# letao1991/EAD-GAN

Measured on NVIDIA B200. Metric: train images/sec (G+D+E step, 64x64 CelebA), higher is better.
Workload: dtype bf16

## Files before the change

eadgan_b200/_lib.py:

```python
from __future__ import annotations

import ctypes as C
import os

import torch

_HERE = os.path.dirname(os.path.abspath(__file__))
LIB_PATH = os.path.join(_HERE, "lib", "libeadgan.so")

ACT_NONE, ACT_RELU, ACT_LRELU, ACT_TANH, ACT_SIGMOID = 0, 1, 2, 3, 4
F32, BF16 = 0, 1
ADAM_MAX_TENSORS = 48


class Tensor4(C.Structure):
    _fields_ = [("ptr", C.c_void_p), ("sn", C.c_int64), ("sc", C.c_int64), ("sh", C.c_int64),
                ("sw", C.c_int64), ("dtype", C.c_int32), ("_pad", C.c_int32)]


class ConvDesc(C.Structure):
    _fields_ = [("n", C.c_int32), ("c", C.c_int32), ("h", C.c_int32), ("w", C.c_int32),
                ("k", C.c_int32), ("r", C.c_int32), ("s", C.c_int32), ("p", C.c_int32),
                ("q", C.c_int32), ("stride", C.c_int32), ("pad", C.c_int32)]


class TcDesc(C.Structure):
    _fields_ = [("n", C.c_int32), ("c", C.c_int32), ("h", C.c_int32), ("w", C.c_int32),
                ("k", C.c_int32), ("act", C.c_int32), ("slope", C.c_float),
                ("out_f32_nchw", C.c_int32), ("want_stats", C.c_int32), ("c_real", C.c_int32),
                ("mask_mode", C.c_int32)]


class AdamTensors(C.Structure):
    _fields_ = [("p", C.c_void_p * ADAM_MAX_TENSORS), ("g", C.c_void_p * ADAM_MAX_TENSORS),
                ("m", C.c_void_p * ADAM_MAX_TENSORS), ("v", C.c_void_p * ADAM_MAX_TENSORS),
                ("numel", C.c_int64 * ADAM_MAX_TENSORS), ("count", C.c_int32), ("_pad", C.c_int32)]


_P = C.c_void_p
_T4 = C.POINTER(Tensor4)
_I, _F, _D, _L = C.c_int, C.c_float, C.c_double, C.c_int64

_PROTOS = {
    "eadgan_conv_fprop": [C.POINTER(ConvDesc), _T4, _P, _P, _I, _F, _T4, _T4, _I, _F, _P],
    "eadgan_conv_dgrad": [C.POINTER(ConvDesc), _T4, _P, _P, _I, _F, _T4, _T4, _I, _F, _P],
    "eadgan_conv_wgrad": [C.POINTER(ConvDesc), _T4, _T4, _P, _P, C.c_size_t, _P],
    "eadgan_channel_sum": [_T4, _I, _I, _I, _I, _P, _P],
    "eadgan_tc_pack_w_fprop": [_P, _P, _I, _I, _I, _P, _P],
    "eadgan_tc_pack_w_dgrad": [_P, _P, _I, _I, _I, _P, _P],
    "eadgan_tc_dense_pack": [_P, _I, _I, _I, _I, _P, _P],
    "eadgan_tc_dense_gather": [_P, _P, _P, _P, _I, _I, _I, _P, C.c_size_t, _P],
    "eadgan_tc_dense_scatter": [_P, _P, _P, _P, _P, _I, _F, _I, _I, _I, _P, _P],
    "eadgan_tc_dense_wgrad": [_P, _P, _P, _P, C.c_size_t, _I, _I, _I, _I, _P],
    "eadgan_tc_fprop": [C.POINTER(TcDesc), _P, _P, _P, _P, _P, _P, _P, _P],
    "eadgan_tc_dgrad": [C.POINTER(TcDesc), _P, _P, _P, _P, _P, _P, _P, _P],
    "eadgan_tc_wgrad": [C.POINTER(TcDesc), _P, _P, _P, _P, C.c_size_t, _P],
    "eadgan_tc_gemm": [_P, _P, _P, _I, _I, _I, _P],
    "eadgan_tc_thin_expand": [_T4, _T4, _I, _F, _I, _I, _I, _I, _P, _P],
    "eadgan_tc_thin_pack_w": [_P, _I, _I, _I, _P, _P],
    "eadgan_tc_thin_fprop": [C.POINTER(TcDesc), _P, _P, _P, _P, _P, _P, _P, _P],
    "eadgan_tc_thin_wgrad": [C.POINTER(TcDesc), _P, _P, _P, _P, C.c_size_t, _P],
    "eadgan_tc_thin_dgrad": [C.POINTER(TcDesc), _P, _P, _P, _P, _P, _P],
    "eadgan_copy4": [_T4, _T4, _I, _I, _I, _I, _P],
    "eadgan_bn_stats": [_T4, _I, _I, _I, _I, _P, _P],
    "eadgan_bn_finalize": [_P, _D, _I, _F, _F, _P, _P, _P, _P, _P],
    "eadgan_bn_apply": [_T4, _I, _I, _I, _I, _P, _P, _P, _P, _I, _F, _T4, _P],
    "eadgan_bn_bwd_reduce": [_T4, _T4, _T4, _I, _I, _I, _I, _P, _P, _P, _P, _I, _F, _P, _P],
    "eadgan_bn_bwd_apply": [_T4, _T4, _T4, _I, _I, _I, _I, _P, _P, _P, _P, _I, _F, _P, _D, _T4, _P],
    "eadgan_bn_bwd_finalize": [_P, _P, _P, _D, _D, _P, _P, _P, _I, _P, _P, _P, _P],
    "eadgan_bn_eval": [_T4, _I, _I, _I, _I, _P, _P, _F, _P, _P, _I, _F, _T4, _P],
    "eadgan_act_fwd": [_P, _P, _L, _I, _F, _P],
    "eadgan_act_bwd": [_P, _P, _P, _L, _I, _F, _P],
    "eadgan_softmax_fwd": [_P, _P, _I, _I, _P],
    "eadgan_softmax_bwd": [_P, _P, _P, _I, _I, _P],
    "eadgan_upsample2x_fwd": [_P, _P, _I, _I, _I, _P],
    "eadgan_upsample2x_bwd": [_P, _P, _I, _I, _I, _P],
    "eadgan_spectral_norm_fwd": [_P, _I, _I, _P, _P, _I, _F, _P, _P, _P, _P],
    "eadgan_spectral_norm_scale": [_P, _P, _P, C.c_longlong, _P],
    "eadgan_spectral_norm_bwd": [_P, _P, _P, _P, _P, _I, _I, _P, _P, _P],
    "eadgan_bce_fwd": [_P, _P, _L, _P, _P],
    "eadgan_bce_bwd": [_P, _P, _P, _L, _P, _P],
    "eadgan_mse_fwd": [_P, _P, _L, _P, _P],
    "eadgan_mse_bwd": [_P, _P, _P, _L, _P, _P, _P],
    "eadgan_ce_fwd": [_P, _P, _I, _I, _P, _P],
    "eadgan_ce_bwd": [_P, _P, _P, _I, _I, _P, _P],
    "eadgan_mi_fwd": [_P, _P, _I, _I, _P, _P],
    "eadgan_mi_bwd": [_P, _P, _P, _I, _I, _P, _P],
    "eadgan_adam_step": [C.POINTER(AdamTensors), _D, _D, _D, _D, _D, _F, _P],
    "eadgan_adam_step_dev": [C.POINTER(AdamTensors), _D, _D, _D, _D, _P, _F, _P],
    "eadgan_adam_advance": [_P, _P],
    "eadgan_fill_f32": [_P, _L, _F, _P],
    "eadgan_f64_to_f32": [_P, _P, _L, _P],
    "eadgan_zero_halo": [_P, _I, _I, _I, _I, _P],
    "eadgan_stn_fwd": [_P, _P, _I, _I, _I, _I, _I, _P, _P],
    "eadgan_affine_grid_fwd": [_P, _I, _I, _I, _P, _P],
    "eadgan_affine_grid_bwd": [_P, _I, _I, _I, _P, _P],
    "eadgan_grid_sample_fwd": [_P, _P, _I, _I, _I, _I, _I, _I, _I, _P, _P],
    "eadgan_grid_sample_bwd": [_P, _P, _P, _I, _I, _I, _I, _I, _I, _I, _P, _P, _P],
    "eadgan_relcode_dims": [_I, _P, _P],
    "eadgan_relcode_fwd": [_I, _P, C.c_longlong, _P, C.c_longlong, _I, _P, _P, _P],
    "eadgan_relcode_bwd": [_I, _P, _P, _I, _P, _P, _P],
    "eadgan_philox": [_I, C.c_ulonglong, _P, C.c_longlong, _I, C.c_longlong, C.c_longlong, C.c_longlong, _F, _F, _I, _P, _P],
}
_SPECIAL = {
    "eadgan_last_error": ([], C.c_char_p),
    "eadgan_version": ([], C.c_int),
    "eadgan_sm_count": ([], C.c_int),
    "eadgan_kernel_launches": ([], C.c_int64),
    "eadgan_tc_workspace_bytes": ([C.POINTER(TcDesc), _I], C.c_size_t),
    "eadgan_conv_wgrad_workspace": ([C.POINTER(ConvDesc)], C.c_size_t),
    "eadgan_tc_thin_buffer_elems": ([_I, _I, _I], C.c_size_t),
    "eadgan_tc_dense_gather_workspace": ([_I], C.c_size_t),
    "eadgan_tc_thin_wgrad_workspace": ([C.POINTER(TcDesc)], C.c_size_t),
    "eadgan_tc_dense_wgrad_workspace": ([_I, _I], C.c_size_t),
    "eadgan_spectral_norm_scratch_floats": ([_I, _I, _I], C.c_size_t),
}
EXPORTED = sorted(list(_PROTOS) + list(_SPECIAL))

weights_epoch = 0


def bump_weights_epoch():
    global weights_epoch
    weights_epoch += 1


step_serial = 0


def next_step_serial():
    global step_serial
    step_serial += 1
    return step_serial


_lib = None
launches = 0


def lib():
    global _lib
    if _lib is None:
        if not os.path.exists(LIB_PATH):
            raise RuntimeError(
                f"{LIB_PATH} is missing: build it with `python -m eadgan_b200.build` "
                "(nvcc, sm_100a). eadgan_b200 has no CPU or cuDNN fallback.")
        l = C.CDLL(LIB_PATH)
        for name, args in _PROTOS.items():
            fn = getattr(l, name)
            fn.argtypes = args
            fn.restype = C.c_int
        for name, (args, res) in _SPECIAL.items():
            fn = getattr(l, name)
            fn.argtypes = args
            fn.restype = res
        _lib = l
    return _lib


_prof = None


def _flops(name, args):
    try:
        d = args[0]._obj
    except AttributeError:
        return 0
    if isinstance(d, ConvDesc):
        return 2 * d.n * d.p * d.q * d.k * d.c * d.r * d.s
    if isinstance(d, TcDesc):
        return 2 * d.n * (d.h // 2) * (d.w // 2) * d.k * d.c * 16
    return 0


def _shape_tag(args):
    try:
        d = args[0]._obj
    except (AttributeError, IndexError):
        return ""
    if isinstance(d, ConvDesc):
        return f"[n{d.n} c{d.c} h{d.h} k{d.k} r{d.r} s{d.stride}]"
    if isinstance(d, TcDesc):
        return f"[n{d.n} c{d.c} h{d.h} k{d.k}]"
    return ""


def profile_start():
    global _prof
    _prof = []


def profile_stop():
    global _prof
    rec, _prof = _prof, None
    torch.cuda.synchronize()
    out = {}
    for name, fl, e0, e1 in rec or []:
        r = out.setdefault(name, {"calls": 0, "ms": 0.0, "flops": 0})
        r["calls"] += 1
        r["ms"] += e0.elapsed_time(e1)
        r["flops"] += fl
    return out


def call(name, *args):
    global launches
    if _prof is not None:
        e0, e1 = torch.cuda.Event(enable_timing=True), torch.cuda.Event(enable_timing=True)
        e0.record()
        rc = getattr(lib(), name)(*args)
        e1.record()
        _prof.append((name + _shape_tag(args), _flops(name, args), e0, e1))
    else:
        rc = getattr(lib(), name)(*args)
    launches += 1
    if rc != 0:
        msg = lib().eadgan_last_error()
        raise RuntimeError(f"{name} failed ({rc}): {msg.decode() if msg else '?'}")


def stream():
    return C.c_void_p(torch.cuda.current_stream().cuda_stream)


def ptr(t):
    return None if t is None else C.c_void_p(t.data_ptr())


def _dt(t):
    if t.dtype == torch.float32:
        return F32
    if t.dtype == torch.bfloat16:
        return BF16
    raise RuntimeError(f"eadgan_b200: unsupported dtype {t.dtype}")


def t4(t: torch.Tensor) -> Tensor4:
    if t.dim() == 2:
        return Tensor4(t.data_ptr(), t.stride(0), t.stride(1), 0, 0, _dt(t), 0)
    assert t.dim() == 4, t.shape
    return Tensor4(t.data_ptr(), t.stride(0), t.stride(1), t.stride(2), t.stride(3), _dt(t), 0)


def require_cuda(t: torch.Tensor, who: str):
    if not t.is_cuda:
        raise RuntimeError(
            f"{who}: eadgan_b200 operators run only on CUDA tensors (sm_100a kernels, no CPU "
            f"fallback); got a {t.device} tensor")
```

eadgan_b200/chain.py:

```python
from __future__ import annotations

import ctypes as C
import os

import torch

from . import _lib as L
from . import functional as Fn
from . import tc
from ._lib import ACT_NONE, call, ptr, stream, t4


def precision():
    return os.environ.get("EADGAN_PRECISION", "bf16")


gate_log = None


def _pow2(v):
    return v > 0 and (v & (v - 1)) == 0


class _Stage:
    __slots__ = ("kind", "conv", "bn", "act", "stride", "pad", "r")

    def __init__(self, kind, conv):
        self.kind, self.conv, self.bn, self.act = kind, conv, None, (ACT_NONE, 0.0)
        self.stride = conv.stride[0]
        self.pad = conv.padding[0]
        self.r = conv.kernel_size[0]


def _compile(seq):
    from . import nn as enn
    mods = list(seq._modules.values())
    stages, i = [], 0
    while i < len(mods):
        m = mods[i]
        if isinstance(m, enn.Conv2d):
            kind = "conv"
        elif isinstance(m, enn.ConvTranspose2d):
            kind = "convT"
        else:
            return None
        if (m.groups != 1 or m.dilation != (1, 1) or m.kernel_size[0] != m.kernel_size[1]
                or m.stride[0] != m.stride[1] or m.padding[0] != m.padding[1] or m._forward_hooks
                or m._backward_hooks or getattr(m, "padding_mode", "zeros") != "zeros"
                or (kind == "convT" and m.output_padding != (0, 0))):
            return None
        st = _Stage(kind, m)
        i += 1
        if i < len(mods) and isinstance(mods[i], enn.BatchNorm2d) and enn._plain(mods[i]):
            bn = mods[i]
            if not (bn.affine and bn.track_running_stats) or bn.momentum is None:
                return None
            st.bn = bn
            i += 1
        if i < len(mods) and isinstance(mods[i], enn._Act) and enn._plain(mods[i]):
            st.act = mods[i].act()
            i += 1
        stages.append(st)
    if not stages or stages[-1].bn is not None:
        return None
    return stages


def _plan(seq):
    key = tuple(id(m) for m in seq._modules.values())
    cached = seq.__dict__.get("_eadgan_plan")
    if cached is None or cached[0] != key:
        cached = (key, _compile(seq))
        seq.__dict__["_eadgan_plan"] = cached
    return cached[1]


_sn_streams = {}
prefetch_enabled = True


def _side_stream(dev):
    side = _sn_streams.get(dev)
    if side is None:
        side = _sn_streams[dev] = torch.cuda.Stream(device=dev)
    side.wait_stream(torch.cuda.current_stream())
    return side


def prefetch_spectral_norm(seq, count=1):
    if precision() != "bf16" or not prefetch_enabled:
        return
    stages = _plan(seq)
    if stages is None:
        return
    convs = [st.conv for st in stages if st.conv._forward_pre_hooks]
    if not convs:
        return
    w0 = getattr(convs[0], "weight_orig", None)
    if w0 is None or not w0.is_cuda:
        return
    side = _side_stream(w0.device)
    with torch.cuda.stream(side):
        for _ in range(count):
            done = []
            Fn.sn_skip_scale = True
            try:
                for conv in convs:
                    conv.__dict__.pop("_eadgan_sn_src", None)
                    for hook in conv._forward_pre_hooks.values():
                        hook(conv, (None,))
                    done.append((conv.weight, conv.__dict__.get("_eadgan_sn_src")))
            finally:
                Fn.sn_skip_scale = False
            ev = torch.cuda.Event()
            ev.record(side)
            for conv, entry in zip(convs, done):
                tag = getattr(getattr(conv, "weight_orig", None), "_eadgan_stepped", 0)
                conv.__dict__.setdefault("_eadgan_sn_queue", []).append((entry, ev, tag))


def prefetch_packs(module):
    if precision() != "bf16" or not prefetch_enabled:
        return
    todo = []
    for seq in module.modules():
        if not isinstance(seq, torch.nn.Sequential):
            continue
        stages = _plan(seq)
        if stages is None:
            continue
        for st in stages:
            p = getattr(st.conv, "weight_orig", None)
            if p is None:
                p = st.conv.weight
            if isinstance(p, torch.nn.Parameter) and p.is_cuda and getattr(p, "_eadgan_pack_uses", None):
                todo.append(p)
    if not todo:
        return
    with torch.cuda.stream(_side_stream(todo[0].device)):
        for p in todo:
            tc.prefetch_packs(p)


def set_trainable(module, flag):
    for p in module.parameters():
        p.requires_grad_(flag)


def clear_prefetch(seq):
    for m in seq._modules.values():
        m.__dict__.pop("_eadgan_sn_queue", None)


def try_run(seq, x):
    if precision() != "bf16" or not torch.is_tensor(x) or not x.is_cuda or x.dim() != 4 or x.dtype != torch.float32:
        return None
    stages = _plan(seq)
    if stages is None:
        return None
    if any(st.bn is not None and not st.bn.training for st in stages):
        return None
    params, srcs = [], []
    for st in stages:
        queue = st.conv.__dict__.get("_eadgan_sn_queue")
        if queue:
            (w_pre, sn_pre), ev, tag = queue.pop(0)
            if tag != getattr(getattr(st.conv, "weight_orig", None), "_eadgan_stepped", 0):
                raise RuntimeError("eadgan_b200.chain: a prefetched spectral-norm result is older than the layer's "
                                   "weights (an optimiser stepped them after prefetch_spectral_norm); the step driver "
                                   "must prefetch only forwards that run before the owning optimiser steps")
            cur = torch.cuda.current_stream()
            cur.wait_event(ev)
            for t in (w_pre,) + (tuple(sn_pre[1:3]) if sn_pre is not None else ()):
                if torch.is_tensor(t):
                    t.record_stream(cur)
            setattr(st.conv, "weight", w_pre)
            if sn_pre is not None:
                st.conv.__dict__["_eadgan_sn_src"] = sn_pre
            else:
                st.conv.__dict__.pop("_eadgan_sn_src", None)
        else:
            st.conv.__dict__.pop("_eadgan_sn_src", None)
            Fn.sn_skip_scale = True
            try:
                for hook in st.conv._forward_pre_hooks.values():
                    hook(st.conv, (x,))
            finally:
                Fn.sn_skip_scale = False
        w = st.conv.weight
        sn = st.conv.__dict__.get("_eadgan_sn_src")
        if sn is not None and sn[2] is w and isinstance(sn[0], torch.nn.Parameter):
            srcs.append((sn[0], sn[1], sn[3]))
        elif sn is not None and sn[3]:
            Fn.spectral_norm_materialize(sn[0], sn[1], sn[2])
            srcs.append(None)
        elif isinstance(w, torch.nn.Parameter):
            srcs.append((w, None))
        else:
            srcs.append(None)
        params += [w, st.conv.bias]
        if st.bn is not None:
            st.bn.num_batches_tracked.add_(1)
            params += [st.bn.weight, st.bn.bias]
    if gate_log is not None:
        gate_log.append((seq, []))
    return _ChainFn.apply(x, stages, srcs, *params)


class _Buf:
    __slots__ = ("t", "fmt")

    def __init__(self, t, fmt):
        self.t, self.fmt = t, fmt

    @property
    def nchw(self):
        if self.fmt == "ext":
            return tuple(self.t.shape)
        n, hp, wp, c = self.t.shape
        return (n, c, hp - 2, wp - 2)

    def view(self):
        return self.t if self.fmt == "ext" else tc.interior(self.t)

    def padded(self):
        return self.t if self.fmt == "pad" else tc.to_padded(self.t)


def _geom(st, in_shape):
    w = st.conv.weight
    r, s_, pad = st.r, st.stride, st.pad
    if st.kind == "conv":
        n, c, h, ww = in_shape
        k = w.shape[0]
        p = (h + 2 * pad - r) // s_ + 1
        q = (ww + 2 * pad - r) // s_ + 1
    else:
        n, k, p, q = in_shape
        c = w.shape[1]
        h = (p - 1) * s_ - 2 * pad + r
        ww = (q - 1) * s_ - 2 * pad + r
    return L.ConvDesc(n, c, h, ww, k, r, r, p, q, s_, pad)


def _calloc(d):
    if d.c % 32 == 0:
        return d.c
    return 32 if d.c < 32 else None


def _tc_ok(d, direction):
    if not (d.r == 4 and d.stride == 2 and d.pad == 1 and d.h == 2 * d.p and d.w == 2 * d.q):
        return False
    if not (_pow2(d.p) and _pow2(d.q)) or _calloc(d) is None:
        return False
    if direction == "fprop":
        return d.k % 32 == 0 and d.q <= 128
    if direction == "dgrad":
        return (d.k % 64 == 0 or d.k == 32) and d.q <= 128
    return d.k % 32 == 0 and d.q <= 64


def _thin_ok(d, direction):
    if not (d.r == 4 and d.stride == 2 and d.pad == 1 and d.h == 2 * d.p and d.w == 2 * d.q and d.c <= 4):
        return False
    if not (_pow2(d.p) and _pow2(d.q)):
        return False
    if direction == "fprop":
        return d.k % 32 == 0 and d.q <= 128
    if direction == "dgrad":
        return (d.k % 64 == 0 or d.k == 32) and d.q == 32 and d.c <= 3
    return d.k % 32 == 0 and d.q <= 64


def _impl(st, d, last):
    unit = d.r == 4 and d.stride == 1 and d.pad == 0 and d.h == 4 and d.w == 4 and d.p == 1 and d.q == 1
    plain = st.bn is None and st.act[0] == ACT_NONE
    if unit and plain and d.c % 128 == 0:
        if st.kind == "convT" and d.k <= 256 and not last:
            return "dense_T"
        if st.kind == "conv" and d.k <= 32 and last:
            return "dense_C"
    direction = "fprop" if st.kind == "conv" else "dgrad"
    if _thin_ok(d, direction) and (st.kind == "conv" or (last and st.bn is None)):
        return "thin"
    if _tc_ok(d, direction):
        if _calloc(d) != d.c and st.kind == "convT" and not (last and st.bn is None):
            return "simt"
        return "tc"
    return "simt"


class _StagePlan:
    __slots__ = ("d", "ca", "fwd", "wgrad", "dx", "fuse", "in_fmt", "out_fmt", "in_shape", "out_shape")


def _plan_kernels(stages, in_shape):
    plans = []
    for si, st in enumerate(stages):
        last, conv = si == len(stages) - 1, st.kind == "conv"
        prev = stages[si - 1] if si > 0 else None
        p = _StagePlan()
        d = p.d = _geom(st, in_shape)
        p.in_shape = tuple(in_shape)
        p.out_shape = (d.n, d.k, d.p, d.q) if conv else (d.n, d.c, d.h, d.w)
        p.fwd = _impl(st, d, last)
        p.ca = _calloc(d) if p.fwd == "tc" else d.c
        if p.fwd in ("dense_T", "dense_C"):
            p.wgrad = "dense"
            p.dx = "dense" if p.fwd == "dense_C" and si > 0 else "simt"
        elif p.fwd == "thin":
            if conv and last:
                raise RuntimeError("eadgan_b200.chain: a thin conv cannot be the last stage")
            p.wgrad = "thin" if _thin_ok(d, "wgrad") else "simt"
            if conv:
                p.dx = "thin" if si == 0 and _thin_ok(d, "dgrad") else "simt"
            else:
                p.dx = "thin" if si > 0 else "simt"
        elif p.fwd == "tc":
            p.wgrad = "tc" if _tc_ok(d, "wgrad") else "simt"
            tc_dx = _tc_ok(d, "dgrad" if conv else "fprop") and not (conv and si > 0 and p.ca != d.c)
            p.dx = "tc" if tc_dx else "simt"
        else:
            p.wgrad = p.dx = "simt"
        p.in_fmt = "ext" if si == 0 and (p.fwd in ("dense_T", "simt") or (p.fwd == "thin" and conv)) else "pad"
        p.out_fmt = "ext" if last else "pad"
        p.fuse = prev is not None and prev.bn is None and prev.act[0] != ACT_NONE
        plans.append(p)
        in_shape = p.out_shape
    return plans


def _chan_sums(buf, c):
    n, cc, h, w = buf.nchw
    if buf.fmt == "ext" and h * w == 1 and cc == c and buf.t.dtype == torch.float32:
        return Fn.channel_sum(buf.t)
    sums = torch.zeros(2 * c, device=buf.t.device, dtype=torch.float64)
    d = t4(buf.view())
    call("eadgan_bn_stats", C.byref(d), n, c, h, w, ptr(sums), stream())
    return sums[:c].float()


def _r64(v):
    return (v + 63) // 64 * 64


class _Arena:

    def __init__(self, n, dev):
        self.buf = torch.zeros(n + 2, device=dev, dtype=torch.float64) if n > 0 else None
        self.off = 0

    def take(self, n):
        n2 = (n + 1) // 2 * 2
        if self.buf is None or self.off + n2 > self.buf.numel():
            return torch.zeros(n, device=self.buf.device if self.buf is not None else "cuda", dtype=torch.float64)
        out = self.buf[self.off:self.off + n]
        self.off += n2
        return out


class _Saved:
    __slots__ = ("w", "src", "lazy", "pi", "has_b", "inp", "y", "R", "a", "pre", "mean", "invstd", "gamma", "beta",
                 "count", "n_local", "sum_x")

    def __init__(self, w, src, pi, has_b):
        self.w, self.src, self.pi, self.has_b = w, src, pi, has_b
        self.lazy = src is not None and len(src) > 2 and bool(src[2])
        self.R = self.a = self.pre = None

    def values(self):
        if self.lazy:
            Fn.spectral_norm_materialize(self.src[0], self.src[1], self.w)
            self.lazy = False
        return self.w.contiguous()

    def packed(self, direction, ca):
        if self.src is not None:
            return tc.pack_w_cached(self.src[0], direction, ca), self.src[1]
        return tc.pack_w(self.values(), None, direction, ca), None

    def packed_thin(self, direction):
        if self.src is not None:
            return tc.thin_pack_w_cached(self.src[0], direction), self.src[1]
        return tc.thin_pack_w(self.values(), direction), None


class _ChainFn(torch.autograd.Function):
    @staticmethod
    def forward(ctx, x, stages, srcs, *params):
        st_ = stream()
        dev = x.device
        plans = _plan_kernels(stages, tuple(x.shape))
        cur = _Buf(x.contiguous(), "ext")
        saved = []
        pi = 0
        arena = _Arena(sum(2 * p.out_shape[1] for st, p in zip(stages, plans) if st.bn is not None), dev)
        for si, (st, p) in enumerate(zip(stages, plans)):
            sv = _Saved(params[pi], srcs[si], pi, params[pi + 1] is not None)
            b = params[pi + 1]
            pi += 4 if st.bn is not None else 2
            d, conv, last = p.d, st.kind == "conv", si == len(stages) - 1
            out_shape = p.out_shape
            cout = out_shape[1]
            epi_act = st.act if st.bn is None else (ACT_NONE, 0.0)
            stats = arena.take(2 * cout) if st.bn is not None else None
            inp = cur if cur.fmt == p.in_fmt else _Buf(tc.to_padded(cur.t, p.ca if conv else None), "pad")
            if p.fwd == "thin" and conv:
                sv.R = tc.thin_expand(inp.view())
                wpk, sg = sv.packed_thin("fprop")
                out_t = tc.thin_fprop(sv.R, wpk, b, d.c, cout, *epi_act, stats=stats, sigma=sg)
            elif p.fwd == "thin":
                wpk, sg = sv.packed_thin("dgrad")
                out_t = tc.thin_dgrad(inp.t, wpk, b, d.c, *epi_act, sigma=sg)
            elif p.fwd == "dense_T":
                sv.a = tc.pad_rows(inp.t.reshape(d.n, d.k), _r64(d.k))
                out_t = tc.dense_scatter(sv.a, tc.dense_pack(sv.values(), _r64(d.k), False), b, d.c)
            elif p.fwd == "dense_C":
                out_t = tc.dense_gather(inp.t, tc.dense_pack(sv.values(), 32, True), b, d.k).view(out_shape)
            elif p.fwd == "tc" and conv:
                wpk, sg = sv.packed("fprop", p.ca)
                out_t = tc.fprop(inp.t, wpk, b, cout, *epi_act, out_f32_nchw=last, stats=stats, sigma=sg)
            elif p.fwd == "tc":
                wpk, sg = sv.packed("dgrad", p.ca)
                out_t = tc.dgrad(inp.t, wpk, b, p.ca, *epi_act, out_f32_nchw=last, stats=stats,
                                 c_real=d.c if p.ca != d.c else 0, sigma=sg)
            else:
                out_t = (torch.empty(out_shape, device=dev, dtype=torch.float32) if last
                         else tc.alloc_padded(out_shape[0], out_shape[2], out_shape[3], cout, dev))
                ind, outd = t4(inp.view()), t4(out_t if last else tc.interior(out_t))
                call("eadgan_conv_fprop" if conv else "eadgan_conv_dgrad", C.byref(d), C.byref(ind),
                     ptr(sv.values()), ptr(b), epi_act[0], float(epi_act[1]), C.byref(outd), None, ACT_NONE, 0.0, st_)
                if stats is not None:
                    call("eadgan_bn_stats", C.byref(outd), out_shape[0], cout, out_shape[2], out_shape[3],
                         ptr(stats), st_)
            out = _Buf(out_t, p.out_fmt)
            sv.inp = inp
            if st.bn is not None:
                bn = st.bn
                gamma, beta = params[pi - 2], params[pi - 1]
                n_local = float(out_shape[0] * out_shape[2] * out_shape[3])
                count = n_local
                sum_x = stats
                if Fn._allreduce_sum is not None:
                    sum_x = stats[:cout].clone()
                    Fn._allreduce_sum(stats)
                    count *= Fn._world_size
                mean = torch.empty(cout, device=dev, dtype=torch.float32)
                invstd = torch.empty(cout, device=dev, dtype=torch.float32)
                call("eadgan_bn_finalize", ptr(stats), count, cout, float(bn.eps), float(bn.momentum), ptr(mean),
                     ptr(invstd), ptr(bn.running_mean), ptr(bn.running_var), st_)
                y = _Buf(tc.alloc_padded(out_shape[0], out_shape[2], out_shape[3], cout, dev), "pad")
                xd, yd = t4(out.view()), t4(y.view())
                call("eadgan_bn_apply", C.byref(xd), out_shape[0], cout, out_shape[2], out_shape[3], ptr(mean),
                     ptr(invstd), ptr(gamma), ptr(beta), st.act[0], float(st.act[1]), C.byref(yd), st_)
                sv.pre, sv.mean, sv.invstd, sv.gamma, sv.beta = out, mean, invstd, gamma, beta
                sv.count, sv.n_local, sv.sum_x = count, n_local, sum_x
                out = y
            sv.y = out
            if gate_log is not None and st.act[0] in (L.ACT_RELU, L.ACT_LRELU):
                gate_log[-1][1].append(out.view() > 0)
            saved.append(sv)
            cur = out
        saved[-1].y = None
        ctx.save_for_backward(cur.t)
        ctx.stages, ctx.plans, ctx.saved = stages, plans, saved
        return cur.t

    @staticmethod
    def backward(ctx, gout):
        stages, plans, saved = ctx.stages, ctx.plans, ctx.saved
        saved[-1].y = _Buf(ctx.saved_tensors[0], "ext")
        st_ = stream()
        dev = gout.device
        g = _Buf(gout.contiguous(), "ext")
        g_masked = False
        db_sums = None
        grads = []
        arena = _Arena(sum(3 * max(p.d.k, p.d.c) for p in plans), dev)
        for si in range(len(stages) - 1, -1, -1):
            st, p, sv = stages[si], plans[si], saved[si]
            d, conv = p.d, st.kind == "conv"
            n, cout, oh, ow = p.out_shape
            dgamma = dbeta = None
            need_dw = ctx.needs_input_grad[3 + sv.pi]
            need_db = sv.has_b and ctx.needs_input_grad[3 + sv.pi + 1]
            need_dx = si > 0 or ctx.needs_input_grad[0]
            if st.bn is not None:
                sums = arena.take(2 * cout)
                gd, xd, yd = t4(g.view()), t4(sv.pre.view()), t4(sv.y.view())
                call("eadgan_bn_bwd_reduce", C.byref(gd), C.byref(xd), C.byref(yd), n, cout, oh, ow, ptr(sv.mean),
                     ptr(sv.invstd), ptr(sv.gamma), ptr(sv.beta), st.act[0], float(st.act[1]), ptr(sums), st_)
                local = sums
                if Fn._allreduce_sum is not None:
                    local = sums.clone()
                    Fn._allreduce_sum(sums)
                call("eadgan_bn_bwd_apply", C.byref(gd), C.byref(xd), C.byref(yd), n, cout, oh, ow, ptr(sv.mean),
                     ptr(sv.invstd), ptr(sv.gamma), ptr(sv.beta), st.act[0], float(st.act[1]), ptr(sums),
                     float(sv.count), C.byref(gd), st_)
                small = torch.empty(3 * cout, device=dev, dtype=torch.float32)
                dgamma, dbeta, db_bn = small[:cout], small[cout:2 * cout], small[2 * cout:]
                call("eadgan_bn_bwd_finalize", ptr(local), ptr(sums), ptr(sv.sum_x), float(sv.n_local),
                     float(sv.count), ptr(sv.mean), ptr(sv.invstd), ptr(sv.gamma), cout, ptr(dgamma),
                     ptr(dbeta), ptr(db_bn) if sv.has_b else None, st_)
                dz = g
            elif st.act[0] != ACT_NONE and not g_masked:
                if g.fmt != "ext" or sv.y.fmt != "ext":
                    raise RuntimeError("eadgan_b200.chain: unfused activation backward on a private buffer")
                dz = _Buf(Fn.act_bwd(g.t, sv.y.t, st.act[0], st.act[1]), "ext")
            else:
                dz = g
            if not need_db:
                db = None
            elif st.bn is not None:
                db = db_bn
            elif db_sums is not None and dz is g:
                db = torch.empty(cout, device=dev, dtype=torch.float32)
                call("eadgan_f64_to_f32", ptr(db_sums), ptr(db), cout, st_)
            else:
                db = _chan_sums(dz, cout)
            db_sums = None
            want_sums = (si > 0 and stages[si - 1].bn is None and saved[si - 1].has_b
                         and ctx.needs_input_grad[3 + saved[si - 1].pi + 1] and p.in_shape[1] <= 1024)
            sums_buf = arena.take(p.in_shape[1]) if want_sums else None
            x_big, dy_small = (sv.inp, dz) if conv else (dz, sv.inp)
            r, a = sv.R, sv.a
            if p.fwd == "thin" and not conv and (need_dw or (need_dx and p.dx == "thin")):
                r = tc.thin_expand(dz.view())
            if p.fwd == "dense_C":
                a = tc.pad_rows(dz.t.reshape(d.n, d.k), 64)
            dw = None
            if not need_dw:
                pass
            elif p.wgrad == "thin":
                dw = tc.thin_wgrad(r, dy_small.padded(), d.c)
            elif p.wgrad == "dense":
                dw = tc.dense_wgrad(a, x_big.padded(), d.k)
            elif p.wgrad == "tc":
                xb = x_big.t if x_big.fmt == "pad" else tc.to_padded(x_big.t, p.ca)
                if not conv and p.ca != d.c:
                    dz = _Buf(xb, "pad")
                dw = tc.wgrad(xb, dy_small.padded(), c_real=d.c if p.ca != d.c else 0)
            else:
                dw = torch.empty_like(sv.w, memory_format=torch.contiguous_format)
                Fn.conv_wgrad(d, t4(x_big.view()), t4(dy_small.view()), dw)
            if need_dx:
                mask = sv.inp.t if p.fuse else None
                mask_act, mask_slope = stages[si - 1].act if p.fuse else (ACT_NONE, 0.0)
                if p.dx == "thin" and conv:
                    wpk, sg = sv.packed_thin("dgrad")
                    dx_t = tc.thin_dgrad(dz.padded(), wpk, None, d.c, sigma=sg)
                elif p.dx == "thin":
                    wpk, sg = sv.packed_thin("fprop")
                    dx_t = tc.thin_fprop(r, wpk, None, d.c, d.k, mask=mask, mask_mode=mask_act, slope=mask_slope,
                                         stats=sums_buf, stats_mode=2, sigma=sg)
                elif p.dx == "dense":
                    dx_t = tc.dense_scatter(a, tc.dense_pack(sv.values(), 64, False), None, d.c, mask=mask,
                                            mask_act=mask_act, slope=mask_slope, chan_sums=sums_buf)
                elif p.dx == "tc" and conv:
                    wpk, sg = sv.packed("dgrad", p.ca)
                    dx_t = tc.dgrad(dz.padded(), wpk, None, p.ca, mask=mask, mask_mode=mask_act, slope=mask_slope,
                                    out_f32_nchw=si == 0, c_real=d.c if p.ca != d.c else 0, stats=sums_buf,
                                    stats_mode=2, sigma=sg)
                elif p.dx == "tc":
                    wpk, sg = sv.packed("fprop", p.ca)
                    dzp = dz.t if dz.fmt == "pad" else tc.to_padded(dz.t, p.ca)
                    dx_t = tc.fprop(dzp, wpk, None, d.k, mask=mask, mask_mode=mask_act, slope=mask_slope,
                                    out_f32_nchw=si == 0, stats=sums_buf, stats_mode=2, sigma=sg)
                else:
                    ic, ih, iw = p.in_shape[1:]
                    dx_t = (tc.alloc_padded(d.n, ih, iw, ic, dev) if si > 0
                            else torch.empty(p.in_shape, device=dev, dtype=torch.float32))
                    dzd, dxd = t4(dz.view()), t4(dx_t if si == 0 else tc.interior(dx_t))
                    md = t4(sv.inp.view()) if p.fuse else None
                    call("eadgan_conv_dgrad" if conv else "eadgan_conv_fprop", C.byref(d), C.byref(dzd),
                         ptr(sv.values()), None, ACT_NONE, 0.0, C.byref(dxd), C.byref(md) if p.fuse else None,
                         mask_act, float(mask_slope), st_)
                g, g_masked = _Buf(dx_t, "ext" if si == 0 else "pad"), p.fuse
                db_sums = sums_buf if p.dx != "simt" else None
            stage_grads = [dw, db]
            if st.bn is not None:
                stage_grads += [dgamma, dbeta]
            grads = stage_grads + grads
        dx0 = g.t if ctx.needs_input_grad[0] else None
        ctx.saved = ctx.plans = None
        return (dx0, None, None, *grads)
```

eadgan_b200/csrc/spectral_norm.cu:

```cuda
#include "common.cuh"

namespace {

__global__ void __launch_bounds__(128) sn_wtu_kernel(const float* __restrict__ W, const float* __restrict__ u,
                                                     float* __restrict__ t, int rows, int cols, int rows_per_blk) {
  const int j = blockIdx.x * 128 + threadIdx.x;
  const int r0 = blockIdx.y * rows_per_blk;
  const int r1 = min(rows, r0 + rows_per_blk);
  if (j >= cols) return;
  float acc = 0.f;
  int i = r0;
  for (; i + 4 <= r1; i += 4) {
    const float a0 = W[(int64_t)i * cols + j], a1 = W[(int64_t)(i + 1) * cols + j];
    const float a2 = W[(int64_t)(i + 2) * cols + j], a3 = W[(int64_t)(i + 3) * cols + j];
    acc = fmaf(a0, u[i], acc); acc = fmaf(a1, u[i + 1], acc);
    acc = fmaf(a2, u[i + 2], acc); acc = fmaf(a3, u[i + 3], acc);
  }
  for (; i < r1; ++i) acc = fmaf(W[(int64_t)i * cols + j], u[i], acc);
  t[(int64_t)blockIdx.y * cols + j] = acc;
}

__global__ void __launch_bounds__(256) sn_vsum_kernel(float* __restrict__ t, int n, int parts, float* __restrict__ nrm) {
  __shared__ float red[32];
  const int i = blockIdx.x * 256 + threadIdx.x;
  float x = 0.f;
  if (i < n) {
    x = t[i];
    for (int p = 1; p < parts; ++p) x += t[(int64_t)p * n + i];
    t[i] = x;
  }
  const float s = eg_block_sum(x * x, red);
  if (threadIdx.x == 0) nrm[blockIdx.x] = s;
}

__global__ void __launch_bounds__(256) sn_wv_kernel(const float* __restrict__ W, const float* __restrict__ x,
                                                    const float* __restrict__ nrm, int nparts, float eps,
                                                    float* __restrict__ v, float* __restrict__ s, int rows, int cols) {
  __shared__ float red[32];
  const int i = blockIdx.x;
  const float* wr = W + (int64_t)i * cols;
  float inv = 1.f;
  if (x != nullptr) {
    float q = 0.f;
    for (int p = 0; p < nparts; ++p) q += nrm[p];
    inv = 1.f / fmaxf(sqrtf(q), eps);
    const int chunk = (cols + rows - 1) / rows;
    for (int j = i * chunk + threadIdx.x; j < min(cols, (i + 1) * chunk); j += blockDim.x) v[j] = x[j] * inv;
  }
  const float* src = x != nullptr ? x : v;
  float acc = 0.f;
  if ((cols & 3) == 0 && ((reinterpret_cast<uintptr_t>(wr) | reinterpret_cast<uintptr_t>(src)) & 15) == 0) {
    for (int j = threadIdx.x; j < (cols >> 2); j += blockDim.x) {
      const float4 a = reinterpret_cast<const float4*>(wr)[j];
      float4 b = reinterpret_cast<const float4*>(src)[j];
      if (x != nullptr) { b.x *= inv; b.y *= inv; b.z *= inv; b.w *= inv; }
      acc = fmaf(a.x, b.x, acc); acc = fmaf(a.y, b.y, acc);
      acc = fmaf(a.z, b.z, acc); acc = fmaf(a.w, b.w, acc);
    }
  } else {
    for (int j = threadIdx.x; j < cols; j += blockDim.x) acc = fmaf(wr[j], x != nullptr ? src[j] * inv : src[j], acc);
  }
  acc = eg_block_sum(acc, red);
  if (threadIdx.x == 0) s[i] = acc;
}

__global__ void __launch_bounds__(1024) sn_sigma_kernel(const float* __restrict__ s, float* __restrict__ u, int rows,
                                                        float eps, int update_u, float* __restrict__ sigma) {
  __shared__ float red[32];
  if (update_u) {
    float q = 0.f;
    for (int i = threadIdx.x; i < rows; i += blockDim.x) q = fmaf(s[i], s[i], q);
    q = eg_block_sum(q, red);
    const float inv = 1.f / fmaxf(sqrtf(q), eps);
    for (int i = threadIdx.x; i < rows; i += blockDim.x) u[i] = s[i] * inv;
    __syncthreads();
  }
  float d = 0.f;
  for (int i = threadIdx.x; i < rows; i += blockDim.x) d = fmaf(u[i], s[i], d);
  d = eg_block_sum(d, red);
  if (threadIdx.x == 0) *sigma = d;
}

__global__ void __launch_bounds__(256) sn_scale_kernel(const float* __restrict__ W, const float* __restrict__ sigma,
                                                       float* __restrict__ out, int64_t n) {
  const float sg = *sigma;
  const int64_t tid = blockIdx.x * (int64_t)blockDim.x + threadIdx.x, nth = (int64_t)gridDim.x * blockDim.x;
  if ((n & 3) == 0 && ((reinterpret_cast<uintptr_t>(W) | reinterpret_cast<uintptr_t>(out)) & 15) == 0) {
    for (int64_t i = tid; i < (n >> 2); i += nth) {
      float4 a = reinterpret_cast<const float4*>(W)[i];
      a.x /= sg; a.y /= sg; a.z /= sg; a.w /= sg;
      reinterpret_cast<float4*>(out)[i] = a;
    }
  } else {
    for (int64_t i = tid; i < n; i += nth) out[i] = W[i] / sg;
  }
}

__global__ void __launch_bounds__(256) sn_dot_kernel(const float* __restrict__ a, const float* __restrict__ b,
                                                     int64_t n, float* __restrict__ part) {
  __shared__ float red[32];
  float s = 0.f;
  if ((n & 3) == 0 && ((reinterpret_cast<uintptr_t>(a) | reinterpret_cast<uintptr_t>(b)) & 15) == 0) {
    for (int64_t i = blockIdx.x * (int64_t)blockDim.x + threadIdx.x; i < (n >> 2); i += (int64_t)gridDim.x * blockDim.x) {
      const float4 x = reinterpret_cast<const float4*>(a)[i], y = reinterpret_cast<const float4*>(b)[i];
      s = fmaf(x.x, y.x, s); s = fmaf(x.y, y.y, s); s = fmaf(x.z, y.z, s); s = fmaf(x.w, y.w, s);
    }
  } else {
    for (int64_t i = blockIdx.x * (int64_t)blockDim.x + threadIdx.x; i < n; i += (int64_t)gridDim.x * blockDim.x)
      s = fmaf(a[i], b[i], s);
  }
  s = eg_block_sum(s, red);
  if (threadIdx.x == 0) part[blockIdx.x] = s;
}

__global__ void __launch_bounds__(256) sn_bwd_kernel(const float* __restrict__ dW, const float* __restrict__ u,
                                                     const float* __restrict__ v, const float* __restrict__ sigma,
                                                     const float* __restrict__ part, int nparts, int rows, int cols,
                                                     float* __restrict__ out) {
  __shared__ float red[32];
  float d = 0.f;
  for (int i = threadIdx.x; i < nparts; i += blockDim.x) d += part[i];
  d = eg_block_sum(d, red);
  const float sg = *sigma;
  const float coef = d / (sg * sg);
  const int64_t n = (int64_t)rows * cols;
  if ((cols & 3) == 0 && ((reinterpret_cast<uintptr_t>(dW) | reinterpret_cast<uintptr_t>(out) | reinterpret_cast<uintptr_t>(v)) & 15) == 0) {
    const int cv = cols >> 2;
    for (int64_t i = blockIdx.x * (int64_t)blockDim.x + threadIdx.x; i < (n >> 2); i += (int64_t)gridDim.x * blockDim.x) {
      const int r = (int)(i / cv), c4 = (int)(i - (int64_t)r * cv);
      const float4 g = reinterpret_cast<const float4*>(dW)[i], vv = reinterpret_cast<const float4*>(v)[c4];
      const float cu = coef * u[r];
      float4 o;
      o.x = g.x / sg - cu * vv.x; o.y = g.y / sg - cu * vv.y; o.z = g.z / sg - cu * vv.z; o.w = g.w / sg - cu * vv.w;
      reinterpret_cast<float4*>(out)[i] = o;
    }
  } else {
    for (int64_t i = blockIdx.x * (int64_t)blockDim.x + threadIdx.x; i < n; i += (int64_t)gridDim.x * blockDim.x) {
      const int r = (int)(i / cols), c = (int)(i - (int64_t)r * cols);
      out[i] = dW[i] / sg - coef * u[r] * v[c];
    }
  }
}

constexpr int SN_SMALL_MAX = 16 * 1024;
constexpr int SN_SMALL_COLS = 4096, SN_SMALL_ROWS = 1024;
__global__ void __launch_bounds__(1024) sn_small_fwd_kernel(const float* __restrict__ W, float* __restrict__ u,
                                                            float* __restrict__ v, int rows, int cols, int do_pi, float eps,
                                                            float* __restrict__ sigma) {
  __shared__ float red[32];
  __shared__ float vs[SN_SMALL_COLS];
  __shared__ float ss[SN_SMALL_ROWS];
  const int tid = threadIdx.x, warp = tid >> 5, lane = tid & 31;
  if (do_pi) {
    for (int i = tid; i < rows; i += 1024) ss[i] = u[i];
    __syncthreads();
    float q = 0.f;
    for (int j = tid; j < cols; j += 1024) {
      float acc = 0.f;
#pragma unroll 8
      for (int i = 0; i < rows; ++i) acc = fmaf(W[(int64_t)i * cols + j], ss[i], acc);
      vs[j] = acc;
      q = fmaf(acc, acc, q);
    }
    q = eg_block_sum(q, red);
    const float inv = 1.f / fmaxf(sqrtf(q), eps);
    for (int j = tid; j < cols; j += 1024) { const float x = vs[j] * inv; vs[j] = x; v[j] = x; }
  } else {
    for (int j = tid; j < cols; j += 1024) vs[j] = v[j];
  }
  __syncthreads();
  for (int i = warp; i < rows; i += 32) {
    const float* wr = W + (int64_t)i * cols;
    float acc = 0.f;
#pragma unroll 8
    for (int j = lane; j < cols; j += 32) acc = fmaf(wr[j], vs[j], acc);
#pragma unroll
    for (int o = 16; o > 0; o >>= 1) acc += __shfl_xor_sync(0xffffffffu, acc, o);
    if (lane == 0) ss[i] = acc;
  }
  __syncthreads();
  if (do_pi) {
    float q = 0.f;
    for (int i = tid; i < rows; i += 1024) q = fmaf(ss[i], ss[i], q);
    q = eg_block_sum(q, red);
    const float inv = 1.f / fmaxf(sqrtf(q), eps);
    float d = 0.f;
    for (int i = tid; i < rows; i += 1024) { const float x = ss[i] * inv; u[i] = x; d = fmaf(x, ss[i], d); }
    d = eg_block_sum(d, red);
    if (tid == 0) *sigma = d;
  } else {
    float d = 0.f;
    for (int i = tid; i < rows; i += 1024) d = fmaf(u[i], ss[i], d);
    d = eg_block_sum(d, red);
    if (tid == 0) *sigma = d;
  }
}

__global__ void __launch_bounds__(1024) sn_small_bwd_kernel(const float* __restrict__ dW, const float* __restrict__ W,
                                                            const float* __restrict__ u, const float* __restrict__ v,
                                                            const float* __restrict__ sigma, int rows, int cols,
                                                            float* __restrict__ out) {
  __shared__ float red[32];
  const int n = rows * cols;
  float d = 0.f;
  for (int i = threadIdx.x; i < n; i += 1024) d = fmaf(dW[i], W[i], d);
  d = eg_block_sum(d, red);
  const float sg = *sigma;
  const float coef = d / (sg * sg);
  for (int i = threadIdx.x; i < n; i += 1024) {
    const int r = i / cols, c = i - r * cols;
    out[i] = dW[i] / sg - coef * u[r] * v[c];
  }
}

bool sn_small(int rows, int cols) {
  return (int64_t)rows * cols <= SN_SMALL_MAX && cols <= SN_SMALL_COLS && rows <= SN_SMALL_ROWS;
}

int grid_for(int64_t n) {
  int64_t b = (n + 1023) / 1024;
  const int64_t cap = 16 * (int64_t)eg_sm_count();
  return (int)(b < 1 ? 1 : (b > cap ? cap : b));
}

}

extern "C" int eadgan_spectral_norm_fwd(const float* w_orig, int rows, int cols, float* u, float* v,
                                        int do_power_iter, float eps, float* sigma, float* w_sn,
                                        float* scratch, void* stream) {
  EG_REQUIRE(w_orig && u && v && sigma && scratch && rows > 0 && cols > 0, EADGAN_ERR_INVALID,
             "spectral_norm_fwd: bad arguments");
  cudaStream_t st = (cudaStream_t)stream;
  if (sn_small(rows, cols)) {
    sn_small_fwd_kernel<<<1, 1024, 0, st>>>(w_orig, u, v, rows, cols, do_power_iter ? 1 : 0, eps, sigma);
    EG_LAUNCH_CHECK("sn_small_fwd_kernel");
    if (w_sn) {
      const int64_t n = (int64_t)rows * cols;
      sn_scale_kernel<<<grid_for(n), 256, 0, st>>>(w_orig, sigma, w_sn, n);
      EG_LAUNCH_CHECK("sn_scale_kernel");
    }
    return 0;
  }
  int col_tiles = (cols + 127) / 128;
  int splits = (4 * eg_sm_count() + col_tiles - 1) / col_tiles;
  int max_splits = (rows + 15) / 16;
  if (splits > max_splits) splits = max_splits;
  if (splits < 1) splits = 1;
  const int rpb = (rows + splits - 1) / splits;
  splits = (rows + rpb - 1) / rpb;
  float* s = scratch;
  float* nrm = scratch + ((rows + 3) & ~3);
  const int nparts = (cols + 255) / 256;
  float* t = nrm + ((nparts + 3) & ~3);
  if (do_power_iter) {
    sn_wtu_kernel<<<dim3(col_tiles, splits), 128, 0, st>>>(w_orig, u, t, rows, cols, rpb);
    EG_LAUNCH_CHECK("sn_wtu_kernel");
    sn_vsum_kernel<<<nparts, 256, 0, st>>>(t, cols, splits, nrm);
    EG_LAUNCH_CHECK("sn_vsum_kernel");
  }
  sn_wv_kernel<<<rows, 256, 0, st>>>(w_orig, do_power_iter ? t : nullptr, nrm, nparts, eps, v, s, rows, cols);
  EG_LAUNCH_CHECK("sn_wv_kernel");
  sn_sigma_kernel<<<1, 1024, 0, st>>>(s, u, rows, eps, do_power_iter ? 1 : 0, sigma);
  EG_LAUNCH_CHECK("sn_sigma_kernel");
  if (w_sn) {
    const int64_t n = (int64_t)rows * cols;
    sn_scale_kernel<<<grid_for(n), 256, 0, st>>>(w_orig, sigma, w_sn, n);
    EG_LAUNCH_CHECK("sn_scale_kernel");
  }
  return 0;
}

extern "C" int eadgan_spectral_norm_bwd(const float* dw_sn, const float* w_orig, const float* u,
                                        const float* v, const float* sigma, int rows, int cols,
                                        float* dw_orig, float* scratch, void* stream) {
  EG_REQUIRE(dw_sn && w_orig && u && v && sigma && dw_orig && scratch && rows > 0 && cols > 0,
             EADGAN_ERR_INVALID, "spectral_norm_bwd: bad arguments");
  cudaStream_t st = (cudaStream_t)stream;
  const int64_t n = (int64_t)rows * cols;
  if (sn_small(rows, cols)) {
    sn_small_bwd_kernel<<<1, 1024, 0, st>>>(dw_sn, w_orig, u, v, sigma, rows, cols, dw_orig);
    EG_LAUNCH_CHECK("sn_small_bwd_kernel");
    return 0;
  }
  const int parts = grid_for(n);
  sn_dot_kernel<<<parts, 256, 0, st>>>(dw_sn, w_orig, n, scratch);
  EG_LAUNCH_CHECK("sn_dot_kernel");
  sn_bwd_kernel<<<grid_for(n), 256, 0, st>>>(dw_sn, u, v, sigma, scratch, parts, rows, cols, dw_orig);
  EG_LAUNCH_CHECK("sn_bwd_kernel");
  return 0;
}

extern "C" size_t eadgan_spectral_norm_scratch_floats(int rows, int cols, int backward) {
  if (backward) return (size_t)grid_for((int64_t)rows * cols) + 8;
  return (size_t)((rows + 3) & ~3) + (size_t)(((cols + 255) / 256 + 3) & ~3) + (size_t)((rows + 15) / 16 + 1) * (size_t)cols + 8;
}

extern "C" int eadgan_spectral_norm_scale(const float* w_orig, const float* sigma, float* w_sn, long long n,
                                          void* stream) {
  EG_REQUIRE(w_orig && sigma && w_sn && n > 0, EADGAN_ERR_INVALID, "spectral_norm_scale: bad arguments");
  sn_scale_kernel<<<grid_for(n), 256, 0, (cudaStream_t)stream>>>(w_orig, sigma, w_sn, n);
  EG_LAUNCH_CHECK("sn_scale_kernel");
  return 0;
}
```

eadgan_b200/functional.py:

```python
from __future__ import annotations

import ctypes as C

import torch

from . import _lib as L
from . import tc
from ._lib import ACT_NONE, ACT_LRELU, ACT_RELU, ACT_SIGMOID, ACT_TANH, call, ptr, stream, t4

_allreduce_sum = None
_world_size = 1


def set_allreduce(fn, world_size):
    global _allreduce_sum, _world_size
    _allreduce_sum, _world_size = fn, int(world_size)


def _f32(t, who):
    L.require_cuda(t, who)
    if t.dtype != torch.float32:
        raise RuntimeError(f"{who}: expected float32, got {t.dtype}")
    return t


def _conv_desc(n, c, h, w, k, r, s, stride, pad):
    p = (h + 2 * pad - r) // stride + 1
    q = (w + 2 * pad - s) // stride + 1
    return L.ConvDesc(n, c, h, w, k, r, s, p, q, stride, pad), p, q


def act_fwd_(x, kind, slope=0.0, out=None):
    out = x if out is None else out
    call("eadgan_act_fwd", ptr(x), ptr(out), x.numel(), kind, float(slope), stream())
    return out


def act_bwd(dy, y, kind, slope=0.0):
    dy = dy.contiguous()
    dx = torch.empty_like(dy)
    call("eadgan_act_bwd", ptr(dy), ptr(y), ptr(dx), dy.numel(), kind, float(slope), stream())
    return dx


def channel_sum(t):
    if t.dim() == 2:
        n, c, h, w = t.shape[0], t.shape[1], 1, 1
    else:
        n, c, h, w = t.shape
    out = torch.empty(c, device=t.device, dtype=torch.float32)
    d = t4(t)
    call("eadgan_channel_sum", C.byref(d), n, c, h, w, ptr(out), stream())
    return out


def conv_wgrad(d, x_t4, dy_t4, dw):
    need = L.lib().eadgan_conv_wgrad_workspace(C.byref(d))
    ws = tc._workspace(need, dw.device) if need else None
    call("eadgan_conv_wgrad", C.byref(d), C.byref(x_t4), C.byref(dy_t4), ptr(dw), ptr(ws),
         C.c_size_t(need), stream())


class _ConvFn(torch.autograd.Function):

    @staticmethod
    def forward(ctx, x, w, b, stride, pad, act, slope):
        _f32(x, "conv2d")
        _f32(w, "conv2d")
        x = x if x.is_contiguous() else x.contiguous()
        w = w.contiguous()
        two_d = x.dim() == 2
        if two_d:
            n, c, h, ww = x.shape[0], x.shape[1], 1, 1
            k, r, s = w.shape[0], 1, 1
        else:
            n, c, h, ww = x.shape
            k, _, r, s = w.shape
        if w.shape[1] != c:
            raise RuntimeError(f"conv2d: weight {tuple(w.shape)} does not match input channels {c}")
        d, p, q = _conv_desc(n, c, h, ww, k, r, s, stride, pad)
        y = torch.empty((n, k) if two_d else (n, k, p, q), device=x.device, dtype=torch.float32)
        xd, yd = t4(x), t4(y)
        call("eadgan_conv_fprop", C.byref(d), C.byref(xd), ptr(w), ptr(b), act, float(slope),
             C.byref(yd), None, ACT_NONE, 0.0, stream())
        ctx.save_for_backward(x, w, y if act != ACT_NONE else None)
        ctx.cfg = (d, act, slope, b is not None)
        return y

    @staticmethod
    def backward(ctx, dy):
        x, w, y = ctx.saved_tensors
        d, act, slope, has_b = ctx.cfg
        dy = dy.contiguous()
        dz = act_bwd(dy, y, act, slope) if act != ACT_NONE else dy
        dx = dw = db = None
        dzd = t4(dz)
        if ctx.needs_input_grad[0]:
            dx = torch.empty_like(x)
            dxd = t4(dx)
            call("eadgan_conv_dgrad", C.byref(d), C.byref(dzd), ptr(w), None, ACT_NONE, 0.0,
                 C.byref(dxd), None, ACT_NONE, 0.0, stream())
        if ctx.needs_input_grad[1]:
            dw = torch.empty_like(w)
            conv_wgrad(d, t4(x), dzd, dw)
        if has_b and ctx.needs_input_grad[2]:
            db = channel_sum(dz)
        return dx, dw, db, None, None, None, None


class _ConvTFn(torch.autograd.Function):

    @staticmethod
    def forward(ctx, x, w, b, stride, pad, act, slope):
        _f32(x, "conv_transpose2d")
        _f32(w, "conv_transpose2d")
        x = x if x.is_contiguous() else x.contiguous()
        w = w.contiguous()
        n, k, p, q = x.shape
        kk, c, r, s = w.shape
        if kk != k:
            raise RuntimeError(f"conv_transpose2d: weight {tuple(w.shape)} does not match input channels {k}")
        h = (p - 1) * stride - 2 * pad + r
        ww = (q - 1) * stride - 2 * pad + s
        d = L.ConvDesc(n, c, h, ww, k, r, s, p, q, stride, pad)
        y = torch.empty((n, c, h, ww), device=x.device, dtype=torch.float32)
        xd, yd = t4(x), t4(y)
        call("eadgan_conv_dgrad", C.byref(d), C.byref(xd), ptr(w), ptr(b), act, float(slope),
             C.byref(yd), None, ACT_NONE, 0.0, stream())
        ctx.save_for_backward(x, w, y if act != ACT_NONE else None)
        ctx.cfg = (d, act, slope, b is not None)
        return y

    @staticmethod
    def backward(ctx, dy):
        x, w, y = ctx.saved_tensors
        d, act, slope, has_b = ctx.cfg
        dy = dy.contiguous()
        dz = act_bwd(dy, y, act, slope) if act != ACT_NONE else dy
        dx = dw = db = None
        dzd = t4(dz)
        if ctx.needs_input_grad[0]:
            dx = torch.empty_like(x)
            dxd = t4(dx)
            call("eadgan_conv_fprop", C.byref(d), C.byref(dzd), ptr(w), None, ACT_NONE, 0.0,
                 C.byref(dxd), None, ACT_NONE, 0.0, stream())
        if ctx.needs_input_grad[1]:
            dw = torch.empty_like(w)
            xd = t4(x)
            conv_wgrad(d, dzd, xd, dw)
        if has_b and ctx.needs_input_grad[2]:
            db = channel_sum(dz)
        return dx, dw, db, None, None, None, None


def conv2d(x, w, b=None, stride=1, padding=0, act=ACT_NONE, slope=0.0):
    return _ConvFn.apply(x, w, b, int(stride), int(padding), act, slope)


def conv_transpose2d(x, w, b=None, stride=1, padding=0, act=ACT_NONE, slope=0.0):
    return _ConvTFn.apply(x, w, b, int(stride), int(padding), act, slope)


def linear(x, w, b=None, act=ACT_NONE, slope=0.0):
    if x.dim() != 2:
        raise RuntimeError("linear: expected a [N, in_features] input")
    return _ConvFn.apply(x, w, b, 1, 0, act, slope)


class _BatchNormFn(torch.autograd.Function):
    @staticmethod
    def forward(ctx, x, gamma, beta, rmean, rvar, training, momentum, eps, act, slope):
        _f32(x, "batch_norm")
        x = x if x.is_contiguous() else x.contiguous()
        n, c, h, w = x.shape
        y = torch.empty_like(x)
        xd, yd = t4(x), t4(y)
        st = stream()
        if not training:
            call("eadgan_bn_eval", C.byref(xd), n, c, h, w, ptr(rmean), ptr(rvar), float(eps), ptr(gamma),
                 ptr(beta), act, float(slope), C.byref(yd), st)
            ctx.training = False
            ctx.save_for_backward(x, gamma, rvar, y)
            ctx.cfg = (eps, act, slope)
            return y
        sums = torch.zeros(2 * c, device=x.device, dtype=torch.float64)
        call("eadgan_bn_stats", C.byref(xd), n, c, h, w, ptr(sums), st)
        count = float(n * h * w)
        if _allreduce_sum is not None:
            _allreduce_sum(sums)
            count *= _world_size
        mean = torch.empty(c, device=x.device, dtype=torch.float32)
        invstd = torch.empty(c, device=x.device, dtype=torch.float32)
        call("eadgan_bn_finalize", ptr(sums), count, c, float(eps), float(momentum), ptr(mean), ptr(invstd),
             ptr(rmean), ptr(rvar), st)
        call("eadgan_bn_apply", C.byref(xd), n, c, h, w, ptr(mean), ptr(invstd), ptr(gamma), ptr(beta), act,
             float(slope), C.byref(yd), st)
        ctx.training = True
        ctx.save_for_backward(x, gamma, beta, mean, invstd, y if act != ACT_NONE else None)
        ctx.cfg = (count, act, slope)
        return y

    @staticmethod
    def backward(ctx, dy):
        dy = dy.contiguous()
        st = stream()
        if not ctx.training:
            x, gamma, rvar, y = ctx.saved_tensors
            raise RuntimeError("batch_norm: backward through eval-mode BatchNorm2d is not on the "
                               "reference's hot path and is not implemented")
        x, gamma, beta, mean, invstd, y = ctx.saved_tensors
        count, act, slope = ctx.cfg
        n, c, h, w = x.shape
        sums = torch.zeros(2 * c, device=x.device, dtype=torch.float64)
        dyd, xd = t4(dy), t4(x)
        yd = t4(y) if y is not None else None
        yref = C.byref(yd) if yd is not None else None
        call("eadgan_bn_bwd_reduce", C.byref(dyd), C.byref(xd), yref, n, c, h, w, ptr(mean), ptr(invstd),
             ptr(gamma), ptr(beta), act, float(slope), ptr(sums), st)
        local = sums.clone() if _allreduce_sum is not None else sums
        if _allreduce_sum is not None:
            _allreduce_sum(sums)
        dx = torch.empty_like(x)
        dxd = t4(dx)
        call("eadgan_bn_bwd_apply", C.byref(dyd), C.byref(xd), yref, n, c, h, w, ptr(mean), ptr(invstd),
             ptr(gamma), ptr(beta), act, float(slope), ptr(sums), count, C.byref(dxd), st)
        dbeta = local[:c].float()
        dgamma = local[c:].float()
        return dx, dgamma, dbeta, None, None, None, None, None, None, None


def batch_norm(x, gamma, beta, rmean, rvar, training, momentum, eps, act=ACT_NONE, slope=0.0):
    return _BatchNormFn.apply(x, gamma, beta, rmean, rvar, bool(training), momentum, eps, act, slope)


class _ActFn(torch.autograd.Function):
    @staticmethod
    def forward(ctx, x, kind, slope, inplace):
        _f32(x, "activation")
        if inplace and x.is_contiguous():
            ctx.mark_dirty(x)
            y = act_fwd_(x, kind, slope)
        else:
            xc = x.contiguous()
            y = torch.empty_like(xc)
            act_fwd_(xc, kind, slope, out=y)
        ctx.save_for_backward(y)
        ctx.cfg = (kind, slope)
        return y

    @staticmethod
    def backward(ctx, dy):
        (y,) = ctx.saved_tensors
        kind, slope = ctx.cfg
        return act_bwd(dy, y, kind, slope), None, None, None


def activation(x, kind, slope=0.0, inplace=False):
    return _ActFn.apply(x, kind, float(slope), bool(inplace))


class _SoftmaxFn(torch.autograd.Function):
    @staticmethod
    def forward(ctx, x):
        _f32(x, "softmax")
        if x.dim() != 2:
            raise RuntimeError("softmax: only [rows, cols] inputs (implicit dim=1) are on the hot path")
        x = x.contiguous()
        y = torch.empty_like(x)
        call("eadgan_softmax_fwd", ptr(x), ptr(y), x.shape[0], x.shape[1], stream())
        ctx.save_for_backward(y)
        return y

    @staticmethod
    def backward(ctx, dy):
        (y,) = ctx.saved_tensors
        dy = dy.contiguous()
        dx = torch.empty_like(y)
        call("eadgan_softmax_bwd", ptr(dy), ptr(y), ptr(dx), y.shape[0], y.shape[1], stream())
        return dx


def softmax(x):
    return _SoftmaxFn.apply(x)


class _Upsample2xFn(torch.autograd.Function):
    @staticmethod
    def forward(ctx, x):
        _f32(x, "upsample")
        x = x.contiguous()
        n, c, h, w = x.shape
        y = torch.empty((n, c, 2 * h, 2 * w), device=x.device, dtype=torch.float32)
        call("eadgan_upsample2x_fwd", ptr(x), ptr(y), n * c, h, w, stream())
        ctx.shape = (n, c, h, w)
        return y

    @staticmethod
    def backward(ctx, dy):
        n, c, h, w = ctx.shape
        dy = dy.contiguous()
        dx = torch.empty((n, c, h, w), device=dy.device, dtype=torch.float32)
        call("eadgan_upsample2x_bwd", ptr(dy), ptr(dx), n * c, h, w, stream())
        return dx


def upsample2x(x):
    return _Upsample2xFn.apply(x)


class _SpectralNormFn(torch.autograd.Function):

    @staticmethod
    def forward(ctx, w_orig, u, v, do_power_iter, eps):
        _f32(w_orig, "spectral_norm")
        w = w_orig.contiguous()
        rows = w.shape[0]
        cols = w.numel() // rows
        sigma = torch.empty(1, device=w.device, dtype=torch.float32)
        w_sn = torch.empty_like(w)
        scratch = torch.empty(L.lib().eadgan_spectral_norm_scratch_floats(rows, cols, 0), device=w.device,
                              dtype=torch.float32)
        call("eadgan_spectral_norm_fwd", ptr(w), rows, cols, ptr(u), ptr(v), 1 if do_power_iter else 0,
             float(eps), ptr(sigma), None if sn_skip_scale else ptr(w_sn), ptr(scratch), stream())
        ctx.mark_non_differentiable(sigma)
        ctx.save_for_backward(w, u.clone(), v.clone(), sigma)
        return w_sn, sigma

    @staticmethod
    def backward(ctx, dw_sn, _dsigma):
        w, u, v, sigma = ctx.saved_tensors
        dw_sn = dw_sn.contiguous()
        rows = w.shape[0]
        cols = w.numel() // rows
        dw = torch.empty_like(w)
        scratch = torch.empty(L.lib().eadgan_spectral_norm_scratch_floats(rows, cols, 1), device=w.device,
                              dtype=torch.float32)
        call("eadgan_spectral_norm_bwd", ptr(dw_sn), ptr(w), ptr(u), ptr(v), ptr(sigma), rows, cols, ptr(dw),
             ptr(scratch), stream())
        return dw, None, None, None, None


sn_skip_scale = False


def spectral_norm_materialize(w_orig, sigma, w_sn):
    call("eadgan_spectral_norm_scale", ptr(w_orig.detach().contiguous()), ptr(sigma), ptr(w_sn), w_sn.numel(), stream())


def spectral_norm_weight(w_orig, u, v, do_power_iter, eps):
    return _SpectralNormFn.apply(w_orig, u, v, bool(do_power_iter), float(eps))


def _same_shape(a, b, who):
    if a.shape != b.shape:
        raise ValueError(f"{who}: input {tuple(a.shape)} and target {tuple(b.shape)} must have the same shape")


class _BCEFn(torch.autograd.Function):
    @staticmethod
    def forward(ctx, p, target):
        _f32(p, "BCELoss")
        _same_shape(p, target, "BCELoss")
        p, target = p.contiguous(), target.contiguous().float()
        loss = torch.empty((), device=p.device, dtype=torch.float32)
        call("eadgan_bce_fwd", ptr(p), ptr(target), p.numel(), ptr(loss), stream())
        ctx.save_for_backward(p, target)
        return loss

    @staticmethod
    def backward(ctx, g):
        p, target = ctx.saved_tensors
        dp = torch.empty_like(p)
        g = g.contiguous().float()
        call("eadgan_bce_bwd", ptr(p), ptr(target), ptr(g), p.numel(), ptr(dp), stream())
        return dp, None


class _MSEFn(torch.autograd.Function):
    @staticmethod
    def forward(ctx, a, b):
        _f32(a, "MSELoss")
        _same_shape(a, b, "MSELoss")
        a, b = a.contiguous(), b.contiguous().float()
        loss = torch.empty((), device=a.device, dtype=torch.float32)
        call("eadgan_mse_fwd", ptr(a), ptr(b), a.numel(), ptr(loss), stream())
        ctx.save_for_backward(a, b)
        return loss

    @staticmethod
    def backward(ctx, g):
        a, b = ctx.saved_tensors
        g = g.contiguous().float()
        da = torch.empty_like(a) if ctx.needs_input_grad[0] else None
        db = torch.empty_like(b) if ctx.needs_input_grad[1] else None
        if da is None and db is None:
            return None, None
        call("eadgan_mse_bwd", ptr(a), ptr(b), ptr(g), a.numel(), ptr(da), ptr(db), stream())
        return da, db


class _CEFn(torch.autograd.Function):
    @staticmethod
    def forward(ctx, x, labels):
        _f32(x, "CrossEntropyLoss")
        if x.dim() != 2 or labels.dim() != 1 or labels.dtype != torch.int64:
            raise RuntimeError("CrossEntropyLoss: expected [N,C] float input and [N] int64 class labels")
        x, labels = x.contiguous(), labels.contiguous()
        loss = torch.empty((), device=x.device, dtype=torch.float32)
        call("eadgan_ce_fwd", ptr(x), ptr(labels), x.shape[0], x.shape[1], ptr(loss), stream())
        ctx.save_for_backward(x, labels)
        return loss

    @staticmethod
    def backward(ctx, g):
        x, labels = ctx.saved_tensors
        g = g.contiguous().float()
        dx = torch.empty_like(x)
        call("eadgan_ce_bwd", ptr(x), ptr(labels), ptr(g), x.shape[0], x.shape[1], ptr(dx), stream())
        return dx, None


class _MIFn(torch.autograd.Function):
    @staticmethod
    def forward(ctx, q, c):
        _f32(q, "mutual_info_loss")
        _same_shape(q, c, "mutual_info_loss")
        q, c = q.contiguous(), c.contiguous().float()
        loss = torch.empty((), device=q.device, dtype=torch.float32)
        call("eadgan_mi_fwd", ptr(q), ptr(c), q.shape[0], q.shape[1], ptr(loss), stream())
        ctx.save_for_backward(q, c)
        return loss

    @staticmethod
    def backward(ctx, g):
        q, c = ctx.saved_tensors
        g = g.contiguous().float()
        dq = torch.empty_like(q)
        call("eadgan_mi_bwd", ptr(q), ptr(c), ptr(g), q.shape[0], q.shape[1], ptr(dq), stream())
        return dq, None


def bce_loss(p, target):
    return _BCEFn.apply(p, target)


def mse_loss(a, b):
    return _MSEFn.apply(a, b)


def cross_entropy(x, labels):
    return _CEFn.apply(x, labels)


def mutual_info_loss(q, c):
    return _MIFn.apply(q, c.detach())


REL_CELEBA, REL_DSPRITES, REL_MNIST = 0, 1, 2
_REL_DIMS = {REL_CELEBA: (5, 5), REL_DSPRITES: (4, 4), REL_MNIST: (7, 6)}


def _rows(t, k, who):
    if not (t.is_cuda and t.dtype == torch.float32 and t.dim() == 2 and t.shape[1] >= k):
        raise RuntimeError(f"{who}: expected a CUDA fp32 [B, >= {k}] tensor")
    if t.stride(1) != 1:
        t = t.contiguous()
    return t, t.stride(0)


class _RelCodeFn(torch.autograd.Function):

    @staticmethod
    def forward(ctx, real, trans, mode):
        k, ko = _REL_DIMS[mode]
        real_k, rs = _rows(real.detach(), k, "relative_code")
        trans_k, ts = _rows(trans.detach(), k, "relative_code")
        n = real.shape[0]
        out = torch.empty((n, ko), device=real.device, dtype=torch.float32)
        jac = torch.empty((n, ko, 2 * k), device=real.device, dtype=torch.float32)
        call("eadgan_relcode_fwd", mode, ptr(real_k), rs, ptr(trans_k), ts, n, ptr(out), ptr(jac), stream())
        ctx.save_for_backward(jac)
        ctx.cfg = (mode, k, real.shape[1], trans.shape[1])
        return out

    @staticmethod
    def backward(ctx, g):
        (jac,) = ctx.saved_tensors
        mode, k, real_w, trans_w = ctx.cfg
        n = jac.shape[0]
        g = g.contiguous()
        d_real = torch.zeros((n, real_w), device=g.device, dtype=torch.float32) if real_w != k else None
        d_trans = torch.zeros((n, trans_w), device=g.device, dtype=torch.float32) if trans_w != k else None
        dr = torch.empty((n, k), device=g.device, dtype=torch.float32)
        dt = torch.empty((n, k), device=g.device, dtype=torch.float32)
        call("eadgan_relcode_bwd", mode, ptr(g), ptr(jac), n, ptr(dr), ptr(dt), stream())
        if d_real is not None:
            d_real[:, :k] = dr
            dr = d_real
        if d_trans is not None:
            d_trans[:, :k] = dt
            dt = d_trans
        return dr, dt, None


def relative_code(real, trans, mode):
    return _RelCodeFn.apply(real, trans, mode)


def stn_fwd(img, theta23, border=True):
    if not (img.is_cuda and img.dtype == torch.float32 and img.dim() == 4):
        raise RuntimeError("stn_fwd: expected a CUDA fp32 [N, C, H, W] image")
    img = img.contiguous()
    theta = theta23.detach().to(torch.float32).contiguous()
    n, c, h, w = img.shape
    if tuple(theta.shape) != (n, 2, 3):
        raise RuntimeError("stn_fwd: theta must be [N, 2, 3]")
    out = torch.empty_like(img)
    call("eadgan_stn_fwd", ptr(img), ptr(theta), n, c, h, w, 1 if border else 0, ptr(out), stream())
    return out


class _AffineGridFn(torch.autograd.Function):
    @staticmethod
    def forward(ctx, theta, n, h, w):
        grid = torch.empty((n, h, w, 2), device=theta.device, dtype=torch.float32)
        call("eadgan_affine_grid_fwd", ptr(theta), n, h, w, ptr(grid), stream())
        ctx.dims = (n, h, w)
        return grid

    @staticmethod
    def backward(ctx, dgrid):
        n, h, w = ctx.dims
        dtheta = torch.empty((n, 2, 3), device=dgrid.device, dtype=torch.float32)
        call("eadgan_affine_grid_bwd", ptr(dgrid.contiguous()), n, h, w, ptr(dtheta), stream())
        return dtheta, None, None, None


def affine_grid(theta, size, align_corners=None):
    if align_corners:
        raise RuntimeError("eadgan_b200 affine_grid: align_corners=True is not used by the reference and unsupported")
    if not (theta.is_cuda and theta.dtype == torch.float32 and theta.dim() == 3 and tuple(theta.shape[1:]) == (2, 3)):
        raise RuntimeError("eadgan_b200 affine_grid: theta must be a CUDA fp32 [N, 2, 3] tensor (no CPU fallback)")
    size = tuple(int(v) for v in size)
    if len(size) != 4 or size[0] != theta.shape[0]:
        raise RuntimeError("eadgan_b200 affine_grid: size must be (N, C, H, W) with N = theta.shape[0]")
    return _AffineGridFn.apply(theta.contiguous(), size[0], size[2], size[3])


class _GridSampleFn(torch.autograd.Function):
    @staticmethod
    def forward(ctx, img, grid, border):
        n, c, h, w = img.shape
        oh, ow = grid.shape[1], grid.shape[2]
        out = torch.empty((n, c, oh, ow), device=img.device, dtype=torch.float32)
        call("eadgan_grid_sample_fwd", ptr(img), ptr(grid), n, c, h, w, oh, ow, int(border), ptr(out), stream())
        ctx.save_for_backward(img, grid)
        ctx.border = int(border)
        return out

    @staticmethod
    def backward(ctx, gout):
        img, grid = ctx.saved_tensors
        n, c, h, w = img.shape
        oh, ow = grid.shape[1], grid.shape[2]
        dimg = torch.zeros_like(img) if ctx.needs_input_grad[0] else None
        dgrid = torch.empty_like(grid) if ctx.needs_input_grad[1] else None
        if dimg is not None or dgrid is not None:
            call("eadgan_grid_sample_bwd", ptr(gout.contiguous()), ptr(img), ptr(grid), n, c, h, w, oh, ow, ctx.border,
                 ptr(dimg), ptr(dgrid), stream())
        return dimg, dgrid, None


def grid_sample(input, grid, mode="bilinear", padding_mode="zeros", align_corners=None):
    if mode != "bilinear" or padding_mode not in ("border", "zeros") or align_corners:
        raise RuntimeError("eadgan_b200 grid_sample: only bilinear, padding_mode 'border' | 'zeros', align_corners=False")
    if not (input.is_cuda and grid.is_cuda and input.dtype == torch.float32 and grid.dtype == torch.float32
            and input.dim() == 4 and grid.dim() == 4 and grid.shape[0] == input.shape[0] and grid.shape[3] == 2):
        raise RuntimeError("eadgan_b200 grid_sample: CUDA fp32 input [N,C,H,W] and grid [N,Ho,Wo,2] required "
                           "(no CPU fallback)")
    return _GridSampleFn.apply(input.contiguous(), grid.contiguous(), padding_mode == "border")
```

eadgan_b200/tc.py:

```python
from __future__ import annotations

import ctypes as C
import weakref

import torch

from . import _lib as L
from ._lib import ACT_NONE, call, ptr, stream, t4


_pool = {}
_pool_enabled = True
capture_births = None


_pool_gen = 0


def _recycle(key, base, gen):
    if gen == _pool_gen:
        _pool.setdefault(key, []).append(base)


def alloc_padded(n, h, w, c, device, zero_interior=False, c_real=None):
    shape = (n, h + 2, w + 2, c)
    if zero_interior or not _pool_enabled:
        return torch.zeros(shape, device=device, dtype=torch.bfloat16)
    key = (shape, c_real or c, str(device))
    free = _pool.get(key)
    if free:
        base = free.pop()
    else:
        base = torch.zeros(shape, device=device, dtype=torch.bfloat16)
        if capture_births is not None:
            capture_births.append(base)
    t = base.view(shape)
    weakref.finalize(t, _recycle, key, base, _pool_gen)
    return t


def clear_pool():
    global _pool_gen
    _pool_gen += 1
    _pool.clear()
    _ws_cache.clear()


def interior(xp):
    n, hp, wp, c = xp.shape
    return xp.permute(0, 3, 1, 2)[:, :, 1:hp - 1, 1:wp - 1]


def to_padded(x, c_alloc=None):
    n, c, h, w = x.shape
    xp = alloc_padded(n, h, w, c_alloc or c, x.device, c_real=c)
    src, dst = t4(x), t4(interior(xp)[:, :c])
    call("eadgan_copy4", C.byref(src), C.byref(dst), n, c, h, w, stream())
    return xp


def pad_rows(x2d, m_pad):
    n, m = x2d.shape
    out = torch.zeros((n, m_pad), device=x2d.device, dtype=torch.bfloat16)
    src, dst = t4(x2d), t4(out[:, :m])
    call("eadgan_copy4", C.byref(src), C.byref(dst), n, m, 1, 1, stream())
    return out


def from_padded(xp, dtype=torch.float32):
    n, hp, wp, c = xp.shape
    out = torch.empty((n, c, hp - 2, wp - 2), device=xp.device, dtype=dtype)
    src, dst = t4(interior(xp)), t4(out)
    call("eadgan_copy4", C.byref(src), C.byref(dst), n, c, hp - 2, wp - 2, stream())
    return out


def pack_w(w, sigma=None, direction="fprop", c_alloc=None):
    k, c = w.shape[0], w.shape[1]
    ca = c_alloc or c
    assert tuple(w.shape[2:]) == (4, 4)
    out = torch.empty(k * 16 * ca, device=w.device, dtype=torch.bfloat16)
    call("eadgan_tc_pack_w_fprop" if direction == "fprop" else "eadgan_tc_pack_w_dgrad",
         ptr(w.contiguous()), ptr(sigma), k, c, ca, ptr(out), stream())
    return out


_pack_cache = {}


def pack_w_cached(param, direction="fprop", c_alloc=None):
    return _cached_pack(param, "wide", direction, c_alloc)


def _cached_pack(param, kind, direction, c_alloc):
    key = (id(param), direction if kind == "wide" else "thin_" + direction, c_alloc)
    token = (param._version, param.data_ptr(), L.weights_epoch, getattr(param, "_eadgan_stepped", 0))
    _note_use(param, kind, direction, c_alloc)
    hit = _pack_cache.get(key)
    if hit is not None and hit[0]() is param and hit[1] == token:
        return _adopt(hit)
    w = param.detach()
    out = thin_pack_w(w, direction) if kind == "thin" else pack_w(w, None, direction, c_alloc)
    if hit is None or hit[0]() is not param:
        weakref.finalize(param, _pack_cache.pop, key, None)
    _pack_cache[key] = (weakref.ref(param), token, out) + _built_on()
    return out


_ahead = False


def _built_on():
    cur = torch.cuda.current_stream()
    ev = None
    if _ahead:
        ev = torch.cuda.Event()
        ev.record(cur)
    return (cur.cuda_stream, ev)


def _adopt(hit):
    if hit[4] is not None:
        cur = torch.cuda.current_stream()
        if cur.cuda_stream != hit[3]:
            cur.wait_event(hit[4])
            hit[2].record_stream(cur)
    return hit[2]


def _note_use(param, kind, direction, c_alloc):
    uses = getattr(param, "_eadgan_pack_uses", None)
    if uses is None:
        uses = set()
        param._eadgan_pack_uses = uses
    uses.add((kind, direction, c_alloc))


def prefetch_packs(param):
    global _ahead
    _ahead = True
    try:
        for kind, direction, c_alloc in tuple(getattr(param, "_eadgan_pack_uses", ())):
            _cached_pack(param, kind, direction, c_alloc)
    finally:
        _ahead = False


def invalidate_caches():
    _pack_cache.clear()
    L.bump_weights_epoch()


def _desc(n, c, h, w, k, act=ACT_NONE, slope=0.0, out_f32_nchw=False, want_stats=False, mask_mode=0, c_real=0):
    return L.TcDesc(n, c, h, w, k, act, float(slope), int(out_f32_nchw), int(want_stats), int(c_real), int(mask_mode))


def fprop(xp, wpk, bias, k, act=ACT_NONE, slope=0.0, out_f32_nchw=False, mask=None, mask_mode=0, stats=None,
          out=None, stats_mode=1, sigma=None):
    n, hp, wp, c = xp.shape
    h, w = hp - 2, wp - 2
    d = _desc(n, c, h, w, k, act, slope, out_f32_nchw, stats_mode if stats is not None else 0, mask_mode)
    if out is None:
        out = (torch.empty((n, k, h // 2, w // 2), device=xp.device, dtype=torch.float32) if out_f32_nchw
               else alloc_padded(n, h // 2, w // 2, k, xp.device))
    call("eadgan_tc_fprop", C.byref(d), ptr(xp), ptr(wpk), ptr(bias), ptr(out), ptr(mask), ptr(stats), ptr(sigma),
         stream())
    return out


def dgrad(yp, wpk, bias, c, act=ACT_NONE, slope=0.0, out_f32_nchw=False, mask=None, mask_mode=0, stats=None,
          out=None, c_real=0, stats_mode=1, sigma=None):
    n, pp, qp, k = yp.shape
    h, w = 2 * (pp - 2), 2 * (qp - 2)
    d = _desc(n, c, h, w, k, act, slope, out_f32_nchw, stats_mode if stats is not None else 0, mask_mode, c_real)
    if out is None:
        out = (torch.empty((n, c_real or c, h, w), device=yp.device, dtype=torch.float32) if out_f32_nchw
               else alloc_padded(n, h, w, c, yp.device))
    call("eadgan_tc_dgrad", C.byref(d), ptr(yp), ptr(wpk), ptr(bias), ptr(out), ptr(mask), ptr(stats), ptr(sigma),
         stream())
    return out


_ws_cache = {}


def _workspace(need, device):
    key = (device, torch.cuda.current_stream().cuda_stream)
    ws = _ws_cache.get(key)
    if ws is None or ws.numel() < need:
        ws = torch.empty(need, device=device, dtype=torch.uint8)
        _ws_cache[key] = ws
    return ws


def dense_pack(w, m_pad, rows_major):
    m, Cc = w.shape[0], w.shape[1]
    out = torch.empty(m_pad * 16 * Cc, device=w.device, dtype=torch.bfloat16)
    call("eadgan_tc_dense_pack", ptr(w.contiguous()), m, m_pad, Cc, 1 if rows_major else 0, ptr(out), stream())
    return out


def dense_gather(yp, w_rows, bias, m_real):
    n, _, _, Cc = yp.shape
    out = torch.empty((n, m_real), device=yp.device, dtype=torch.float32)
    ws = _workspace(L.lib().eadgan_tc_dense_gather_workspace(n), yp.device)
    call("eadgan_tc_dense_gather", ptr(yp), ptr(w_rows), ptr(bias), ptr(out), n, Cc, m_real, ptr(ws),
         C.c_size_t(ws.numel()), stream())
    return out


def dense_scatter(a, w_cols, bias, Cc, mask=None, mask_act=0, slope=0.0, chan_sums=None):
    n, m_pad = a.shape
    out = alloc_padded(n, 4, 4, Cc, a.device)
    call("eadgan_tc_dense_scatter", ptr(a), ptr(w_cols), ptr(bias), ptr(out), ptr(mask), int(mask_act), float(slope),
         n, Cc, m_pad, ptr(chan_sums), stream())
    return out


def dense_wgrad(a, yp, m_real):
    n, m_pad = a.shape
    Cc = yp.shape[3]
    need = L.lib().eadgan_tc_dense_wgrad_workspace(Cc, m_pad)
    ws = _workspace(need, a.device)
    dw = torch.empty((m_real, Cc, 4, 4), device=a.device, dtype=torch.float32)
    call("eadgan_tc_dense_wgrad", ptr(a), ptr(yp), ptr(dw), ptr(ws), C.c_size_t(ws.numel()), n, Cc, m_real, m_pad,
         stream())
    return dw


def wgrad(xp, yp, c_real=0):
    n, hp, wp, c = xp.shape
    k = yp.shape[3]
    d = _desc(n, c, hp - 2, wp - 2, k, c_real=c_real)
    need = L.lib().eadgan_tc_workspace_bytes(C.byref(d), 2)
    if need == 0:
        raise RuntimeError(f"tc wgrad: unsupported geometry n={n} c={c} h={hp - 2} k={k}")
    ws = _workspace(need, xp.device)
    dw = torch.empty((k, c_real or c, 4, 4), device=xp.device, dtype=torch.float32)
    call("eadgan_tc_wgrad", C.byref(d), ptr(xp), ptr(yp), ptr(dw), ptr(ws), C.c_size_t(ws.numel()), stream())
    return dw


def thin_expand(x, mask_y=None, act=ACT_NONE, slope=0.0):
    n, c, h, w = x.shape
    r = torch.empty((n, h // 2, w + 2, 4, 4), device=x.device, dtype=torch.bfloat16)
    src = t4(x)
    mk = t4(mask_y) if mask_y is not None else None
    call("eadgan_tc_thin_expand", C.byref(src), C.byref(mk) if mk is not None else None, int(act), float(slope), n, c, h, w,
         ptr(r), stream())
    return r


def thin_pack_w(w, direction):
    k, c = w.shape[0], w.shape[1]
    assert tuple(w.shape[2:]) == (4, 4) and c <= 4
    out = torch.empty(k * 64, device=w.device, dtype=torch.bfloat16)
    call("eadgan_tc_thin_pack_w", ptr(w.contiguous()), k, c, 0 if direction == "fprop" else 1, ptr(out), stream())
    return out


def thin_pack_w_cached(param, direction):
    return _cached_pack(param, "thin", direction, None)


def thin_fprop(r, wpk, bias, c, k, act=ACT_NONE, slope=0.0, mask=None, mask_mode=0, stats=None, stats_mode=1, sigma=None,
               out=None):
    n, p, wp = r.shape[0], r.shape[1], r.shape[2]
    h, w = 2 * p, wp - 2
    d = _desc(n, c, h, w, k, act, slope, False, stats_mode if stats is not None else 0, mask_mode)
    if out is None:
        out = alloc_padded(n, h // 2, w // 2, k, r.device)
    call("eadgan_tc_thin_fprop", C.byref(d), ptr(r), ptr(wpk), ptr(bias), ptr(out), ptr(mask), ptr(stats), ptr(sigma),
         stream())
    return out


def thin_wgrad(r, yp, c):
    n, p, wp = r.shape[0], r.shape[1], r.shape[2]
    k = yp.shape[3]
    d = _desc(n, c, 2 * p, wp - 2, k)
    need = L.lib().eadgan_tc_thin_wgrad_workspace(C.byref(d))
    if need == 0:
        raise RuntimeError(f"tc thin wgrad: unsupported geometry n={n} c={c} h={2 * p} k={k}")
    ws = _workspace(need, r.device)
    dw = torch.empty((k, c, 4, 4), device=r.device, dtype=torch.float32)
    call("eadgan_tc_thin_wgrad", C.byref(d), ptr(r), ptr(yp), ptr(dw), ptr(ws), C.c_size_t(ws.numel()), stream())
    return dw


def thin_dgrad(yp, wpk, bias, c, act=ACT_NONE, slope=0.0, sigma=None, out=None):
    n, pp, qp, k = yp.shape
    h, w = 2 * (pp - 2), 2 * (qp - 2)
    d = _desc(n, c, h, w, k, act, slope, True)
    if out is None:
        out = torch.empty((n, c, h, w), device=yp.device, dtype=torch.float32)
    call("eadgan_tc_thin_dgrad", C.byref(d), ptr(yp), ptr(wpk), ptr(bias), ptr(out), ptr(sigma), stream())
    return out


def gemm(a, b):
    m, kk = a.shape
    n = b.shape[0]
    c = torch.empty((m, n), device=a.device, dtype=torch.float32)
    call("eadgan_tc_gemm", ptr(a.contiguous()), ptr(b.contiguous()), ptr(c), m, n, kk, stream())
    return c
```

include/eadgan.h:

```cpp
#ifndef EADGAN_H_
#define EADGAN_H_

#include <stddef.h>
#include <stdint.h>

#ifdef __cplusplus
extern "C" {
#endif

#define EADGAN_VERSION 100

typedef enum {
  EADGAN_OK = 0,
  EADGAN_ERR_INVALID = -1,
  EADGAN_ERR_UNSUPPORTED = -2,
  EADGAN_ERR_CUDA = -3,
  EADGAN_ERR_WORKSPACE = -4
} eadgan_status;

typedef enum { EADGAN_F32 = 0, EADGAN_BF16 = 1 } eadgan_dtype;

typedef enum {
  EADGAN_ACT_NONE = 0,
  EADGAN_ACT_RELU = 1,
  EADGAN_ACT_LRELU = 2,
  EADGAN_ACT_TANH = 3,
  EADGAN_ACT_SIGMOID = 4
} eadgan_act;

typedef struct {
  void* ptr;
  int64_t sn, sc, sh, sw;
  int32_t dtype;
  int32_t _pad;
} eadgan_tensor4;

typedef struct {
  int32_t n, c, h, w;
  int32_t k, r, s;
  int32_t p, q;
  int32_t stride, pad;
} eadgan_conv_desc;

const char* eadgan_last_error(void);
int eadgan_version(void);
int eadgan_sm_count(void);
int64_t eadgan_kernel_launches(void);

int eadgan_conv_fprop(const eadgan_conv_desc* d, const eadgan_tensor4* x, const float* w,
                      const float* bias, int act, float slope, const eadgan_tensor4* y,
                      const eadgan_tensor4* mask, int mask_act, float mask_slope, void* stream);
int eadgan_conv_dgrad(const eadgan_conv_desc* d, const eadgan_tensor4* dy, const float* w,
                      const float* bias, int act, float slope, const eadgan_tensor4* dx,
                      const eadgan_tensor4* mask, int mask_act, float mask_slope, void* stream);
size_t eadgan_conv_wgrad_workspace(const eadgan_conv_desc* d);
int eadgan_conv_wgrad(const eadgan_conv_desc* d, const eadgan_tensor4* x, const eadgan_tensor4* dy,
                      float* dw, void* workspace, size_t ws_bytes, void* stream);
int eadgan_channel_sum(const eadgan_tensor4* t, int n, int c, int h, int w, float* out,
                       void* stream);

typedef struct {
  int32_t n, c, h, w;
  int32_t k;
  int32_t act;
  float slope;
  int32_t out_f32_nchw;
  int32_t want_stats;
  int32_t c_real;
  int32_t mask_mode;
} eadgan_tc_desc;

int eadgan_tc_pack_w_fprop(const float* w, const float* sigma, int k, int c_real, int c,
                           void* w_packed, void* stream);
int eadgan_tc_pack_w_dgrad(const float* w, const float* sigma, int k, int c_real, int c,
                           void* w_packed, void* stream);
size_t eadgan_tc_workspace_bytes(const eadgan_tc_desc* d, int direction);
int eadgan_tc_fprop(const eadgan_tc_desc* d, const void* x_pad, const void* w_packed,
                    const float* bias, void* y, const void* mask, double* stats, const float* sigma,
                    void* stream);
int eadgan_tc_dgrad(const eadgan_tc_desc* d, const void* dy_pad, const void* w_packed,
                    const float* bias, void* dx, const void* mask, double* stats, const float* sigma,
                    void* stream);
int eadgan_tc_wgrad(const eadgan_tc_desc* d, const void* x_pad, const void* dy_pad, float* dw,
                    void* workspace, size_t ws_bytes, void* stream);
int eadgan_tc_gemm(const void* a_bf16, const void* b_bf16, float* c_f32, int m, int n, int kk,
                   void* stream);

size_t eadgan_tc_thin_buffer_elems(int n, int h, int w);
int eadgan_tc_thin_expand(const eadgan_tensor4* src, const eadgan_tensor4* mask, int act, float slope,
                          int n, int c_real, int h, int w, void* r_out, void* stream);
int eadgan_tc_thin_pack_w(const float* w, int k, int c_real, int direction, void* out, void* stream);
int eadgan_tc_thin_fprop(const eadgan_tc_desc* d, const void* r_buf, const void* w_packed,
                         const float* bias, void* y, const void* mask, double* stats, const float* sigma,
                         void* stream);
size_t eadgan_tc_thin_wgrad_workspace(const eadgan_tc_desc* d);
int eadgan_tc_thin_wgrad(const eadgan_tc_desc* d, const void* r_buf, const void* dy_pad, float* dw,
                         void* workspace, size_t ws_bytes, void* stream);
int eadgan_tc_thin_dgrad(const eadgan_tc_desc* d, const void* dy_pad, const void* w_packed,
                         const float* bias, float* out, const float* sigma, void* stream);

int eadgan_tc_dense_pack(const float* w, int m_real, int m_pad, int C, int rows_major, void* out,
                         void* stream);
size_t eadgan_tc_dense_gather_workspace(int n);
int eadgan_tc_dense_gather(const void* y_pad, const void* w_rows, const float* bias, float* out, int n,
                           int C, int m_real, void* workspace, size_t ws_bytes, void* stream);
int eadgan_tc_dense_scatter(const void* a_bf16, const void* w_cols, const float* bias, void* out_pad,
                            const void* mask, int mask_act, float slope, int n, int C, int m_pad,
                            double* chan_sums ,
                            void* stream);
size_t eadgan_tc_dense_wgrad_workspace(int C, int m_pad);
int eadgan_tc_dense_wgrad(const void* a_bf16, const void* y_pad, float* dw, void* workspace,
                          size_t ws_bytes, int n, int C, int m_real, int m_pad, void* stream);

int eadgan_copy4(const eadgan_tensor4* src, const eadgan_tensor4* dst, int n, int c, int h, int w,
                 void* stream);

int eadgan_bn_stats(const eadgan_tensor4* x, int n, int c, int h, int w, double* sums, void* stream);
int eadgan_bn_finalize(const double* sums, double count, int c, float eps, float momentum,
                       float* mean, float* invstd, float* running_mean, float* running_var,
                       void* stream);
int eadgan_bn_apply(const eadgan_tensor4* x, int n, int c, int h, int w, const float* mean,
                    const float* invstd, const float* gamma, const float* beta, int act, float slope,
                    const eadgan_tensor4* y, void* stream);
int eadgan_bn_bwd_reduce(const eadgan_tensor4* dy, const eadgan_tensor4* x, const eadgan_tensor4* y,
                         int n, int c, int h, int w, const float* mean, const float* invstd,
                         const float* gamma, const float* beta, int act, float slope, double* sums,
                         void* stream);
int eadgan_bn_bwd_apply(const eadgan_tensor4* dy, const eadgan_tensor4* x, const eadgan_tensor4* y,
                        int n, int c, int h, int w, const float* mean, const float* invstd,
                        const float* gamma, const float* beta, int act, float slope,
                        const double* sums, double count, const eadgan_tensor4* dx, void* stream);
int eadgan_bn_bwd_finalize(const double* local_sums, const double* global_sums,
                           const double* fwd_local_sum_x, double n_local, double count,
                           const float* mean, const float* invstd, const float* gamma, int c,
                           float* dgamma, float* dbeta, float* dbias, void* stream);
int eadgan_bn_eval(const eadgan_tensor4* x, int n, int c, int h, int w, const float* running_mean,
                   const float* running_var, float eps, const float* gamma, const float* beta,
                   int act, float slope, const eadgan_tensor4* y, void* stream);

int eadgan_act_fwd(const float* x, float* y, int64_t numel, int act, float slope, void* stream);
int eadgan_act_bwd(const float* dy, const float* y, float* dx, int64_t numel, int act, float slope,
                   void* stream);
int eadgan_softmax_fwd(const float* x, float* y, int rows, int cols, void* stream);
int eadgan_softmax_bwd(const float* dy, const float* y, float* dx, int rows, int cols, void* stream);
int eadgan_upsample2x_fwd(const float* x, float* y, int nc, int h, int w, void* stream);
int eadgan_upsample2x_bwd(const float* dy, float* dx, int nc, int h, int w, void* stream);

size_t eadgan_spectral_norm_scratch_floats(int rows, int cols, int backward);
int eadgan_spectral_norm_fwd(const float* w_orig, int rows, int cols, float* u, float* v,
                             int do_power_iter, float eps, float* sigma, float* w_sn,
                             float* scratch, void* stream);
int eadgan_spectral_norm_scale(const float* w_orig, const float* sigma, float* w_sn, long long n, void* stream);
int eadgan_spectral_norm_bwd(const float* dw_sn, const float* w_orig, const float* u,
                             const float* v, const float* sigma, int rows, int cols,
                             float* dw_orig, float* scratch, void* stream);

int eadgan_bce_fwd(const float* p, const float* target, int64_t numel, float* loss, void* stream);
int eadgan_bce_bwd(const float* p, const float* target, const float* gout, int64_t numel,
                   float* dp, void* stream);
int eadgan_mse_fwd(const float* a, const float* b, int64_t numel, float* loss, void* stream);
int eadgan_mse_bwd(const float* a, const float* b, const float* gout, int64_t numel, float* da,
                   float* db, void* stream);
int eadgan_ce_fwd(const float* x, const int64_t* labels, int rows, int cols, float* loss,
                  void* stream);
int eadgan_ce_bwd(const float* x, const int64_t* labels, const float* gout, int rows, int cols,
                  float* dx, void* stream);
int eadgan_mi_fwd(const float* q, const float* c, int rows, int cols, float* loss, void* stream);
int eadgan_mi_bwd(const float* q, const float* c, const float* gout, int rows, int cols, float* dq,
                  void* stream);

#define EADGAN_ADAM_MAX_TENSORS 48
typedef struct {
  float* p[EADGAN_ADAM_MAX_TENSORS];
  const float* g[EADGAN_ADAM_MAX_TENSORS];
  float* m[EADGAN_ADAM_MAX_TENSORS];
  float* v[EADGAN_ADAM_MAX_TENSORS];
  int64_t numel[EADGAN_ADAM_MAX_TENSORS];
  int32_t count;
  int32_t _pad;
} eadgan_adam_tensors;
int eadgan_adam_step(const eadgan_adam_tensors* t, double beta1, double beta2, double eps,
                     double step_size, double bc2_sqrt, float grad_scale, void* stream);
int eadgan_adam_step_dev(const eadgan_adam_tensors* t, double beta1, double beta2, double eps, double lr,
                         const int64_t* step_dev, float grad_scale, void* stream);
int eadgan_adam_advance(int64_t* step_dev, void* stream);

int eadgan_fill_f32(float* p, int64_t numel, float value, void* stream);
int eadgan_f64_to_f32(const double* src, float* dst, int64_t numel, void* stream);
int eadgan_zero_halo(void* xp, int n, int h, int w, int c, void* stream);

int eadgan_stn_fwd(const float* img, const float* theta, int n, int c, int h, int w, int padding_border,
                   float* out, void* stream);
int eadgan_affine_grid_fwd(const float* theta, int n, int h, int w, float* grid, void* stream);
int eadgan_affine_grid_bwd(const float* dgrid, int n, int h, int w, float* dtheta, void* stream);
int eadgan_grid_sample_fwd(const float* img, const float* grid, int n, int c, int h, int w, int oh, int ow,
                           int padding_border, float* out, void* stream);
int eadgan_grid_sample_bwd(const float* gout, const float* img, const float* grid, int n, int c, int h, int w, int oh,
                           int ow, int padding_border, float* dimg_zeroed, float* dgrid, void* stream);
int eadgan_relcode_dims(int mode, int* k_in, int* k_out);
int eadgan_relcode_fwd(int mode, const float* real, long long real_stride, const float* trans,
                       long long trans_stride, int n, float* out, float* jac, void* stream);
int eadgan_relcode_bwd(int mode, const float* g, const float* jac, int n, float* d_real, float* d_trans,
                       void* stream);

int eadgan_philox(int kind, unsigned long long seed, const int64_t* step_dev, long long step_host, int stream_id,
                  long long row0, long long rows, long long cols, float lo, float hi, int n, void* out, void* stream);

#ifdef __cplusplus
}
#endif
#endif
```

Baseline: 49630.

## Batch spectral-norm power iterations across layers and cache dense weight packs

Replaces the per-layer spectral-norm forward, which ran several small kernels per layer per step, with a multi-layer grouped launch. A per-launch layer table is indexed by block id, so one kernel launch covers all layers, and several future steps' u/v/sigma can be prefetched at once on a side stream. It also routes dense-path weight packing through the existing pack cache so unchanged weights are not repacked. The cost is more intricate block-to-layer mapping, an extra copy of u/v per step, and new workspace management.

```diff
diff --git a/eadgan_b200/_lib.py b/eadgan_b200/_lib.py
--- a/eadgan_b200/_lib.py
+++ b/eadgan_b200/_lib.py
@@ -35,6 +35,11 @@
     _fields_ = [("p", C.c_void_p * ADAM_MAX_TENSORS), ("g", C.c_void_p * ADAM_MAX_TENSORS),
                 ("m", C.c_void_p * ADAM_MAX_TENSORS), ("v", C.c_void_p * ADAM_MAX_TENSORS),
                 ("numel", C.c_int64 * ADAM_MAX_TENSORS), ("count", C.c_int32), ("_pad", C.c_int32)]
+
+
+class SnLayer(C.Structure):
+    _fields_ = [("w", C.c_void_p), ("rows", C.c_int32), ("cols", C.c_int32), ("u", C.c_void_p), ("v", C.c_void_p),
+                ("u_out", C.c_void_p), ("v_out", C.c_void_p), ("sigma_out", C.c_void_p)]
 
 
 _P = C.c_void_p
@@ -75,7 +80,7 @@
     "eadgan_softmax_bwd": [_P, _P, _P, _I, _I, _P],
     "eadgan_upsample2x_fwd": [_P, _P, _I, _I, _I, _P],
     "eadgan_upsample2x_bwd": [_P, _P, _I, _I, _I, _P],
-    "eadgan_spectral_norm_fwd": [_P, _I, _I, _P, _P, _I, _F, _P, _P, _P, _P],
+    "eadgan_spectral_norm_fwd_multi": [C.POINTER(SnLayer), _I, _I, _I, _F, _P, C.c_size_t, _P],
     "eadgan_spectral_norm_scale": [_P, _P, _P, C.c_longlong, _P],
     "eadgan_spectral_norm_bwd": [_P, _P, _P, _P, _P, _I, _I, _P, _P, _P],
     "eadgan_bce_fwd": [_P, _P, _L, _P, _P],
@@ -114,6 +119,7 @@
     "eadgan_tc_thin_wgrad_workspace": ([C.POINTER(TcDesc)], C.c_size_t),
     "eadgan_tc_dense_wgrad_workspace": ([_I, _I], C.c_size_t),
     "eadgan_spectral_norm_scratch_floats": ([_I, _I, _I], C.c_size_t),
+    "eadgan_spectral_norm_fwd_workspace": ([C.POINTER(SnLayer), _I], C.c_size_t),
 }
 EXPORTED = sorted(list(_PROTOS) + list(_SPECIAL))
 
diff --git a/eadgan_b200/chain.py b/eadgan_b200/chain.py
--- a/eadgan_b200/chain.py
+++ b/eadgan_b200/chain.py
@@ -96,27 +96,32 @@
     convs = [st.conv for st in stages if st.conv._forward_pre_hooks]
     if not convs:
         return
-    w0 = getattr(convs[0], "weight_orig", None)
-    if w0 is None or not w0.is_cuda:
+    from . import nn as enn
+    hooks = [h for conv in convs for h in conv._forward_pre_hooks.values()]
+    if (len(hooks) != len(convs) or not all(isinstance(h, enn.SpectralNorm) and h.name == "weight" for h in hooks)
+            or len({h.eps for h in hooks}) != 1 or not all(conv.training for conv in convs)):
+        return
+    w0 = convs[0].weight_orig
+    if not w0.is_cuda:
         return
     side = _side_stream(w0.device)
     with torch.cuda.stream(side):
-        for _ in range(count):
-            done = []
-            Fn.sn_skip_scale = True
-            try:
-                for conv in convs:
-                    conv.__dict__.pop("_eadgan_sn_src", None)
-                    for hook in conv._forward_pre_hooks.values():
-                        hook(conv, (None,))
-                    done.append((conv.weight, conv.__dict__.get("_eadgan_sn_src")))
-            finally:
-                Fn.sn_skip_scale = False
-            ev = torch.cuda.Event()
-            ev.record(side)
-            for conv, entry in zip(convs, done):
-                tag = getattr(getattr(conv, "weight_orig", None), "_eadgan_stepped", 0)
-                conv.__dict__.setdefault("_eadgan_sn_queue", []).append((entry, ev, tag))
+        res = Fn.spectral_norm_forwards([(c.weight_orig, c.weight_u, c.weight_v) for c in convs], count, True,
+                                        hooks[0].eps)
+        entries = [[] for _ in convs]
+        Fn.sn_skip_scale = True
+        try:
+            for i in range(count):
+                for ent, conv, (us, vs, sg) in zip(entries, convs, res):
+                    w_sn = Fn.spectral_norm_apply(conv.weight_orig, us[i], vs[i], sg[i:i + 1])
+                    ent.append((w_sn, (conv.weight_orig, sg[i:i + 1], w_sn, True)))
+        finally:
+            Fn.sn_skip_scale = False
+        ev = torch.cuda.Event()
+        ev.record(side)
+    for conv, ent in zip(convs, entries):
+        tag = getattr(conv.weight_orig, "_eadgan_stepped", 0)
+        conv.__dict__.setdefault("_eadgan_sn_queue", []).extend((e, ev, tag) for e in ent)
 
 
 def prefetch_packs(module):
@@ -380,6 +385,11 @@
             return tc.pack_w_cached(self.src[0], direction, ca), self.src[1]
         return tc.pack_w(self.values(), None, direction, ca), None
 
+    def dense(self, m_pad, rows_major):
+        if self.src is not None and self.src[1] is None:
+            return tc.dense_pack_cached(self.src[0], m_pad, rows_major)
+        return tc.dense_pack(self.values(), m_pad, rows_major)
+
     def packed_thin(self, direction):
         if self.src is not None:
             return tc.thin_pack_w_cached(self.src[0], direction), self.src[1]
@@ -415,9 +425,9 @@
                 out_t = tc.thin_dgrad(inp.t, wpk, b, d.c, *epi_act, sigma=sg)
             elif p.fwd == "dense_T":
                 sv.a = tc.pad_rows(inp.t.reshape(d.n, d.k), _r64(d.k))
-                out_t = tc.dense_scatter(sv.a, tc.dense_pack(sv.values(), _r64(d.k), False), b, d.c)
+                out_t = tc.dense_scatter(sv.a, sv.dense(_r64(d.k), False), b, d.c)
             elif p.fwd == "dense_C":
-                out_t = tc.dense_gather(inp.t, tc.dense_pack(sv.values(), 32, True), b, d.k).view(out_shape)
+                out_t = tc.dense_gather(inp.t, sv.dense(32, True), b, d.k).view(out_shape)
             elif p.fwd == "tc" and conv:
                 wpk, sg = sv.packed("fprop", p.ca)
                 out_t = tc.fprop(inp.t, wpk, b, cout, *epi_act, out_f32_nchw=last, stats=stats, sigma=sg)
@@ -555,7 +565,7 @@
                     dx_t = tc.thin_fprop(r, wpk, None, d.c, d.k, mask=mask, mask_mode=mask_act, slope=mask_slope,
                                          stats=sums_buf, stats_mode=2, sigma=sg)
                 elif p.dx == "dense":
-                    dx_t = tc.dense_scatter(a, tc.dense_pack(sv.values(), 64, False), None, d.c, mask=mask,
+                    dx_t = tc.dense_scatter(a, sv.dense(64, False), None, d.c, mask=mask,
                                             mask_act=mask_act, slope=mask_slope, chan_sums=sums_buf)
                 elif p.dx == "tc" and conv:
                     wpk, sg = sv.packed("dgrad", p.ca)
diff --git a/eadgan_b200/csrc/spectral_norm.cu b/eadgan_b200/csrc/spectral_norm.cu
--- a/eadgan_b200/csrc/spectral_norm.cu
+++ b/eadgan_b200/csrc/spectral_norm.cu
@@ -1,85 +1,6 @@
 #include "common.cuh"
 
 namespace {
-
-__global__ void __launch_bounds__(128) sn_wtu_kernel(const float* __restrict__ W, const float* __restrict__ u,
-                                                     float* __restrict__ t, int rows, int cols, int rows_per_blk) {
-  const int j = blockIdx.x * 128 + threadIdx.x;
-  const int r0 = blockIdx.y * rows_per_blk;
-  const int r1 = min(rows, r0 + rows_per_blk);
-  if (j >= cols) return;
-  float acc = 0.f;
-  int i = r0;
-  for (; i + 4 <= r1; i += 4) {
-    const float a0 = W[(int64_t)i * cols + j], a1 = W[(int64_t)(i + 1) * cols + j];
-    const float a2 = W[(int64_t)(i + 2) * cols + j], a3 = W[(int64_t)(i + 3) * cols + j];
-    acc = fmaf(a0, u[i], acc); acc = fmaf(a1, u[i + 1], acc);
-    acc = fmaf(a2, u[i + 2], acc); acc = fmaf(a3, u[i + 3], acc);
-  }
-  for (; i < r1; ++i) acc = fmaf(W[(int64_t)i * cols + j], u[i], acc);
-  t[(int64_t)blockIdx.y * cols + j] = acc;
-}
-
-__global__ void __launch_bounds__(256) sn_vsum_kernel(float* __restrict__ t, int n, int parts, float* __restrict__ nrm) {
-  __shared__ float red[32];
-  const int i = blockIdx.x * 256 + threadIdx.x;
-  float x = 0.f;
-  if (i < n) {
-    x = t[i];
-    for (int p = 1; p < parts; ++p) x += t[(int64_t)p * n + i];
-    t[i] = x;
-  }
-  const float s = eg_block_sum(x * x, red);
-  if (threadIdx.x == 0) nrm[blockIdx.x] = s;
-}
-
-__global__ void __launch_bounds__(256) sn_wv_kernel(const float* __restrict__ W, const float* __restrict__ x,
-                                                    const float* __restrict__ nrm, int nparts, float eps,
-                                                    float* __restrict__ v, float* __restrict__ s, int rows, int cols) {
-  __shared__ float red[32];
-  const int i = blockIdx.x;
-  const float* wr = W + (int64_t)i * cols;
-  float inv = 1.f;
-  if (x != nullptr) {
-    float q = 0.f;
-    for (int p = 0; p < nparts; ++p) q += nrm[p];
-    inv = 1.f / fmaxf(sqrtf(q), eps);
-    const int chunk = (cols + rows - 1) / rows;
-    for (int j = i * chunk + threadIdx.x; j < min(cols, (i + 1) * chunk); j += blockDim.x) v[j] = x[j] * inv;
-  }
-  const float* src = x != nullptr ? x : v;
-  float acc = 0.f;
-  if ((cols & 3) == 0 && ((reinterpret_cast<uintptr_t>(wr) | reinterpret_cast<uintptr_t>(src)) & 15) == 0) {
-    for (int j = threadIdx.x; j < (cols >> 2); j += blockDim.x) {
-      const float4 a = reinterpret_cast<const float4*>(wr)[j];
-      float4 b = reinterpret_cast<const float4*>(src)[j];
-      if (x != nullptr) { b.x *= inv; b.y *= inv; b.z *= inv; b.w *= inv; }
-      acc = fmaf(a.x, b.x, acc); acc = fmaf(a.y, b.y, acc);
-      acc = fmaf(a.z, b.z, acc); acc = fmaf(a.w, b.w, acc);
-    }
-  } else {
-    for (int j = threadIdx.x; j < cols; j += blockDim.x) acc = fmaf(wr[j], x != nullptr ? src[j] * inv : src[j], acc);
-  }
-  acc = eg_block_sum(acc, red);
-  if (threadIdx.x == 0) s[i] = acc;
-}
-
-__global__ void __launch_bounds__(1024) sn_sigma_kernel(const float* __restrict__ s, float* __restrict__ u, int rows,
-                                                        float eps, int update_u, float* __restrict__ sigma) {
-  __shared__ float red[32];
-  if (update_u) {
-    float q = 0.f;
-    for (int i = threadIdx.x; i < rows; i += blockDim.x) q = fmaf(s[i], s[i], q);
-    q = eg_block_sum(q, red);
-    const float inv = 1.f / fmaxf(sqrtf(q), eps);
-    for (int i = threadIdx.x; i < rows; i += blockDim.x) u[i] = s[i] * inv;
-    __syncthreads();
-  }
-  float d = 0.f;
-  for (int i = threadIdx.x; i < rows; i += blockDim.x) d = fmaf(u[i], s[i], d);
-  d = eg_block_sum(d, red);
-  if (threadIdx.x == 0) *sigma = d;
-}
 
 __global__ void __launch_bounds__(256) sn_scale_kernel(const float* __restrict__ W, const float* __restrict__ sigma,
                                                        float* __restrict__ out, int64_t n) {
@@ -144,13 +65,160 @@
 
 constexpr int SN_SMALL_MAX = 16 * 1024;
 constexpr int SN_SMALL_COLS = 4096, SN_SMALL_ROWS = 1024;
-__global__ void __launch_bounds__(1024) sn_small_fwd_kernel(const float* __restrict__ W, float* __restrict__ u,
-                                                            float* __restrict__ v, int rows, int cols, int do_pi, float eps,
-                                                            float* __restrict__ sigma) {
+
+__global__ void __launch_bounds__(1024) sn_small_bwd_kernel(const float* __restrict__ dW, const float* __restrict__ W,
+                                                            const float* __restrict__ u, const float* __restrict__ v,
+                                                            const float* __restrict__ sigma, int rows, int cols,
+                                                            float* __restrict__ out) {
+  __shared__ float red[32];
+  const int n = rows * cols;
+  float d = 0.f;
+  for (int i = threadIdx.x; i < n; i += 1024) d = fmaf(dW[i], W[i], d);
+  d = eg_block_sum(d, red);
+  const float sg = *sigma;
+  const float coef = d / (sg * sg);
+  for (int i = threadIdx.x; i < n; i += 1024) {
+    const int r = i / cols, c = i - r * cols;
+    out[i] = dW[i] / sg - coef * u[r] * v[c];
+  }
+}
+
+bool sn_small(int rows, int cols) {
+  return (int64_t)rows * cols <= SN_SMALL_MAX && cols <= SN_SMALL_COLS && rows <= SN_SMALL_ROWS;
+}
+
+int grid_for(int64_t n) {
+  int64_t b = (n + 1023) / 1024;
+  const int64_t cap = 16 * (int64_t)eg_sm_count();
+  return (int)(b < 1 ? 1 : (b > cap ? cap : b));
+}
+
+constexpr int SN_MAX_LAYERS = 16;
+
+struct SnDev {
+  const float* w;
+  float *u, *v;
+  float *u_out, *v_out, *sigma_out;
+  float *s, *nrm, *t;
+  int rows, cols, small, col_tiles, splits, rpb, nparts;
+  int b_wtu, b_vsum, b_wv;
+};
+struct SnTab {
+  SnDev l[SN_MAX_LAYERS];
+  int n;
+};
+
+template <int SnDev::*FIRST>
+__device__ __forceinline__ int sn_layer(const SnTab& tab) {
+  int li = 0;
+  while (li + 1 < tab.n && (int)blockIdx.x >= tab.l[li + 1].*FIRST) ++li;
+  return li;
+}
+
+__global__ void __launch_bounds__(128) sn_wtu_kernel(SnTab tab) {
+  const SnDev& L = tab.l[sn_layer<&SnDev::b_wtu>(tab)];
+  const int b = blockIdx.x - L.b_wtu, cols = L.cols;
+  const int j = (b % L.col_tiles) * 128 + threadIdx.x, split = b / L.col_tiles;
+  const int r0 = split * L.rpb, r1 = min(L.rows, r0 + L.rpb);
+  if (j >= cols) return;
+  const float *W = L.w, *u = L.u;
+  float acc = 0.f;
+  int i = r0;
+  for (; i + 4 <= r1; i += 4) {
+    const float a0 = W[(int64_t)i * cols + j], a1 = W[(int64_t)(i + 1) * cols + j];
+    const float a2 = W[(int64_t)(i + 2) * cols + j], a3 = W[(int64_t)(i + 3) * cols + j];
+    acc = fmaf(a0, u[i], acc); acc = fmaf(a1, u[i + 1], acc);
+    acc = fmaf(a2, u[i + 2], acc); acc = fmaf(a3, u[i + 3], acc);
+  }
+  for (; i < r1; ++i) acc = fmaf(W[(int64_t)i * cols + j], u[i], acc);
+  L.t[(int64_t)split * cols + j] = acc;
+}
+
+__global__ void __launch_bounds__(256) sn_vsum_kernel(SnTab tab) {
+  __shared__ float red[32];
+  const SnDev& L = tab.l[sn_layer<&SnDev::b_vsum>(tab)];
+  const int b = blockIdx.x - L.b_vsum, n = L.cols;
+  const int i = b * 256 + threadIdx.x;
+  float* t = L.t;
+  float x = 0.f;
+  if (i < n) {
+    x = t[i];
+    for (int p = 1; p < L.splits; ++p) x += t[(int64_t)p * n + i];
+    t[i] = x;
+  }
+  const float s = eg_block_sum(x * x, red);
+  if (threadIdx.x == 0) L.nrm[b] = s;
+}
+
+__global__ void __launch_bounds__(256) sn_wv_kernel(SnTab tab, int do_pi, float eps, int f) {
+  __shared__ float red[32];
+  const SnDev& L = tab.l[sn_layer<&SnDev::b_wv>(tab)];
+  const int i = blockIdx.x - L.b_wv, rows = L.rows, cols = L.cols;
+  const float* wr = L.w + (int64_t)i * cols;
+  const float* x = do_pi ? L.t : nullptr;
+  float* v = L.v;
+  float* vo = L.v_out + (int64_t)f * cols;
+  float inv = 1.f;
+  const int chunk = (cols + rows - 1) / rows;
+  if (x != nullptr) {
+    float q = 0.f;
+    for (int p = 0; p < L.nparts; ++p) q += L.nrm[p];
+    inv = 1.f / fmaxf(sqrtf(q), eps);
+    for (int j = i * chunk + threadIdx.x; j < min(cols, (i + 1) * chunk); j += blockDim.x) {
+      const float val = x[j] * inv;
+      v[j] = val;
+      vo[j] = val;
+    }
+  } else {
+    for (int j = i * chunk + threadIdx.x; j < min(cols, (i + 1) * chunk); j += blockDim.x) vo[j] = v[j];
+  }
+  const float* src = x != nullptr ? x : v;
+  float acc = 0.f;
+  if ((cols & 3) == 0 && ((reinterpret_cast<uintptr_t>(wr) | reinterpret_cast<uintptr_t>(src)) & 15) == 0) {
+    for (int j = threadIdx.x; j < (cols >> 2); j += blockDim.x) {
+      const float4 a = reinterpret_cast<const float4*>(wr)[j];
+      float4 b = reinterpret_cast<const float4*>(src)[j];
+      if (x != nullptr) { b.x *= inv; b.y *= inv; b.z *= inv; b.w *= inv; }
+      acc = fmaf(a.x, b.x, acc); acc = fmaf(a.y, b.y, acc);
+      acc = fmaf(a.z, b.z, acc); acc = fmaf(a.w, b.w, acc);
+    }
+  } else {
+    for (int j = threadIdx.x; j < cols; j += blockDim.x) acc = fmaf(wr[j], x != nullptr ? src[j] * inv : src[j], acc);
+  }
+  acc = eg_block_sum(acc, red);
+  if (threadIdx.x == 0) L.s[i] = acc;
+}
+
+__global__ void __launch_bounds__(1024) sn_sigma_kernel(SnTab tab, int do_pi, float eps, int f) {
   __shared__ float red[32];
   __shared__ float vs[SN_SMALL_COLS];
   __shared__ float ss[SN_SMALL_ROWS];
-  const int tid = threadIdx.x, warp = tid >> 5, lane = tid & 31;
+  const SnDev& L = tab.l[blockIdx.x];
+  const int rows = L.rows, cols = L.cols, tid = threadIdx.x;
+  float *u = L.u, *v = L.v;
+  float* uo = L.u_out + (int64_t)f * rows;
+  float* vo = L.v_out + (int64_t)f * cols;
+  float* sigma = L.sigma_out + f;
+  if (!L.small) {
+    const float* s = L.s;
+    if (do_pi) {
+      float q = 0.f;
+      for (int i = tid; i < rows; i += blockDim.x) q = fmaf(s[i], s[i], q);
+      q = eg_block_sum(q, red);
+      const float inv = 1.f / fmaxf(sqrtf(q), eps);
+      for (int i = tid; i < rows; i += blockDim.x) { u[i] = s[i] * inv; uo[i] = s[i] * inv; }
+      __syncthreads();
+    } else {
+      for (int i = tid; i < rows; i += blockDim.x) uo[i] = u[i];
+    }
+    float d = 0.f;
+    for (int i = tid; i < rows; i += blockDim.x) d = fmaf(u[i], s[i], d);
+    d = eg_block_sum(d, red);
+    if (tid == 0) *sigma = d;
+    return;
+  }
+  const float* W = L.w;
+  const int warp = tid >> 5, lane = tid & 31;
   if (do_pi) {
     for (int i = tid; i < rows; i += 1024) ss[i] = u[i];
     __syncthreads();
@@ -164,9 +232,9 @@
     }
     q = eg_block_sum(q, red);
     const float inv = 1.f / fmaxf(sqrtf(q), eps);
-    for (int j = tid; j < cols; j += 1024) { const float x = vs[j] * inv; vs[j] = x; v[j] = x; }
-  } else {
-    for (int j = tid; j < cols; j += 1024) vs[j] = v[j];
+    for (int j = tid; j < cols; j += 1024) { const float x = vs[j] * inv; vs[j] = x; v[j] = x; vo[j] = x; }
+  } else {
+    for (int j = tid; j < cols; j += 1024) { vs[j] = v[j]; vo[j] = v[j]; }
   }
   __syncthreads();
   for (int i = warp; i < rows; i += 32) {
@@ -185,87 +253,94 @@
     q = eg_block_sum(q, red);
     const float inv = 1.f / fmaxf(sqrtf(q), eps);
     float d = 0.f;
-    for (int i = tid; i < rows; i += 1024) { const float x = ss[i] * inv; u[i] = x; d = fmaf(x, ss[i], d); }
+    for (int i = tid; i < rows; i += 1024) { const float x = ss[i] * inv; u[i] = x; uo[i] = x; d = fmaf(x, ss[i], d); }
     d = eg_block_sum(d, red);
     if (tid == 0) *sigma = d;
   } else {
     float d = 0.f;
-    for (int i = tid; i < rows; i += 1024) d = fmaf(u[i], ss[i], d);
+    for (int i = tid; i < rows; i += 1024) { d = fmaf(u[i], ss[i], d); uo[i] = u[i]; }
     d = eg_block_sum(d, red);
     if (tid == 0) *sigma = d;
   }
 }
 
-__global__ void __launch_bounds__(1024) sn_small_bwd_kernel(const float* __restrict__ dW, const float* __restrict__ W,
-                                                            const float* __restrict__ u, const float* __restrict__ v,
-                                                            const float* __restrict__ sigma, int rows, int cols,
-                                                            float* __restrict__ out) {
-  __shared__ float red[32];
-  const int n = rows * cols;
-  float d = 0.f;
-  for (int i = threadIdx.x; i < n; i += 1024) d = fmaf(dW[i], W[i], d);
-  d = eg_block_sum(d, red);
-  const float sg = *sigma;
-  const float coef = d / (sg * sg);
-  for (int i = threadIdx.x; i < n; i += 1024) {
-    const int r = i / cols, c = i - r * cols;
-    out[i] = dW[i] / sg - coef * u[r] * v[c];
-  }
-}
-
-bool sn_small(int rows, int cols) {
-  return (int64_t)rows * cols <= SN_SMALL_MAX && cols <= SN_SMALL_COLS && rows <= SN_SMALL_ROWS;
-}
-
-int grid_for(int64_t n) {
-  int64_t b = (n + 1023) / 1024;
-  const int64_t cap = 16 * (int64_t)eg_sm_count();
-  return (int)(b < 1 ? 1 : (b > cap ? cap : b));
-}
-
-}
-
-extern "C" int eadgan_spectral_norm_fwd(const float* w_orig, int rows, int cols, float* u, float* v,
-                                        int do_power_iter, float eps, float* sigma, float* w_sn,
-                                        float* scratch, void* stream) {
-  EG_REQUIRE(w_orig && u && v && sigma && scratch && rows > 0 && cols > 0, EADGAN_ERR_INVALID,
-             "spectral_norm_fwd: bad arguments");
+void sn_splits(int rows, int cols, int* col_tiles, int* splits, int* rpb) {
+  *col_tiles = (cols + 127) / 128;
+  int sp = (4 * eg_sm_count() + *col_tiles - 1) / *col_tiles;
+  const int max_splits = (rows + 15) / 16;
+  if (sp > max_splits) sp = max_splits;
+  if (sp < 1) sp = 1;
+  *rpb = (rows + sp - 1) / sp;
+  *splits = (rows + *rpb - 1) / *rpb;
+}
+
+size_t sn_r4(int64_t n) { return (size_t)((n + 3) & ~(int64_t)3); }
+
+size_t sn_layer_floats(int rows, int cols) {
+  if (sn_small(rows, cols)) return 0;
+  int col_tiles, splits, rpb;
+  sn_splits(rows, cols, &col_tiles, &splits, &rpb);
+  return sn_r4(rows) + sn_r4((cols + 255) / 256) + sn_r4((int64_t)splits * cols);
+}
+
+}
+
+extern "C" size_t eadgan_spectral_norm_fwd_workspace(const EadganSnLayer* layers, int n) {
+  size_t f = 0;
+  for (int i = 0; i < n; ++i) f += sn_layer_floats(layers[i].rows, layers[i].cols);
+  return f * sizeof(float);
+}
+
+extern "C" int eadgan_spectral_norm_fwd_multi(const EadganSnLayer* layers, int n, int count, int do_power_iter,
+                                              float eps, void* ws, size_t ws_bytes, void* stream) {
+  EG_REQUIRE(layers && n > 0 && count > 0 && (do_power_iter || count == 1), EADGAN_ERR_INVALID,
+             "spectral_norm_fwd_multi: bad arguments");
+  EG_REQUIRE(ws_bytes >= eadgan_spectral_norm_fwd_workspace(layers, n) && ((uintptr_t)ws & 15) == 0,
+             EADGAN_ERR_INVALID, "spectral_norm_fwd_multi: workspace too small or misaligned");
   cudaStream_t st = (cudaStream_t)stream;
-  if (sn_small(rows, cols)) {
-    sn_small_fwd_kernel<<<1, 1024, 0, st>>>(w_orig, u, v, rows, cols, do_power_iter ? 1 : 0, eps, sigma);
-    EG_LAUNCH_CHECK("sn_small_fwd_kernel");
-    if (w_sn) {
-      const int64_t n = (int64_t)rows * cols;
-      sn_scale_kernel<<<grid_for(n), 256, 0, st>>>(w_orig, sigma, w_sn, n);
-      EG_LAUNCH_CHECK("sn_scale_kernel");
-    }
-    return 0;
-  }
-  int col_tiles = (cols + 127) / 128;
-  int splits = (4 * eg_sm_count() + col_tiles - 1) / col_tiles;
-  int max_splits = (rows + 15) / 16;
-  if (splits > max_splits) splits = max_splits;
-  if (splits < 1) splits = 1;
-  const int rpb = (rows + splits - 1) / splits;
-  splits = (rows + rpb - 1) / rpb;
-  float* s = scratch;
-  float* nrm = scratch + ((rows + 3) & ~3);
-  const int nparts = (cols + 255) / 256;
-  float* t = nrm + ((nparts + 3) & ~3);
-  if (do_power_iter) {
-    sn_wtu_kernel<<<dim3(col_tiles, splits), 128, 0, st>>>(w_orig, u, t, rows, cols, rpb);
-    EG_LAUNCH_CHECK("sn_wtu_kernel");
-    sn_vsum_kernel<<<nparts, 256, 0, st>>>(t, cols, splits, nrm);
-    EG_LAUNCH_CHECK("sn_vsum_kernel");
-  }
-  sn_wv_kernel<<<rows, 256, 0, st>>>(w_orig, do_power_iter ? t : nullptr, nrm, nparts, eps, v, s, rows, cols);
-  EG_LAUNCH_CHECK("sn_wv_kernel");
-  sn_sigma_kernel<<<1, 1024, 0, st>>>(s, u, rows, eps, do_power_iter ? 1 : 0, sigma);
-  EG_LAUNCH_CHECK("sn_sigma_kernel");
-  if (w_sn) {
-    const int64_t n = (int64_t)rows * cols;
-    sn_scale_kernel<<<grid_for(n), 256, 0, st>>>(w_orig, sigma, w_sn, n);
-    EG_LAUNCH_CHECK("sn_scale_kernel");
+  float* f = (float*)ws;
+  for (int g0 = 0; g0 < n; g0 += SN_MAX_LAYERS) {
+    SnTab tab;
+    tab.n = n - g0 < SN_MAX_LAYERS ? n - g0 : SN_MAX_LAYERS;
+    int b_wtu = 0, b_vsum = 0, b_wv = 0;
+    for (int i = 0; i < tab.n; ++i) {
+      const EadganSnLayer& a = layers[g0 + i];
+      EG_REQUIRE(a.w && a.u && a.v && a.u_out && a.v_out && a.sigma_out && a.rows > 0 && a.cols > 0,
+                 EADGAN_ERR_INVALID, "spectral_norm_fwd_multi: bad layer %d", g0 + i);
+      SnDev& L = tab.l[i];
+      L.w = a.w; L.u = a.u; L.v = a.v; L.u_out = a.u_out; L.v_out = a.v_out; L.sigma_out = a.sigma_out;
+      L.rows = a.rows; L.cols = a.cols;
+      L.small = sn_small(a.rows, a.cols) ? 1 : 0;
+      L.s = L.nrm = L.t = nullptr;
+      L.col_tiles = L.splits = L.rpb = L.nparts = 0;
+      if (!L.small) {
+        sn_splits(a.rows, a.cols, &L.col_tiles, &L.splits, &L.rpb);
+        L.nparts = (a.cols + 255) / 256;
+        L.s = f; f += sn_r4(a.rows);
+        L.nrm = f; f += sn_r4(L.nparts);
+        L.t = f; f += sn_r4((int64_t)L.splits * a.cols);
+      }
+      L.b_wtu = b_wtu; L.b_vsum = b_vsum; L.b_wv = b_wv;
+      if (!L.small) {
+        b_wtu += L.col_tiles * L.splits;
+        b_vsum += L.nparts;
+        b_wv += a.rows;
+      }
+    }
+    for (int fw = 0; fw < count; ++fw) {
+      if (b_wv > 0) {
+        if (do_power_iter) {
+          sn_wtu_kernel<<<b_wtu, 128, 0, st>>>(tab);
+          EG_LAUNCH_CHECK("sn_wtu_kernel");
+          sn_vsum_kernel<<<b_vsum, 256, 0, st>>>(tab);
+          EG_LAUNCH_CHECK("sn_vsum_kernel");
+        }
+        sn_wv_kernel<<<b_wv, 256, 0, st>>>(tab, do_power_iter, eps, fw);
+        EG_LAUNCH_CHECK("sn_wv_kernel");
+      }
+      sn_sigma_kernel<<<tab.n, 1024, 0, st>>>(tab, do_power_iter, eps, fw);
+      EG_LAUNCH_CHECK("sn_sigma_kernel");
+    }
   }
   return 0;
 }
@@ -291,8 +366,7 @@
 }
 
 extern "C" size_t eadgan_spectral_norm_scratch_floats(int rows, int cols, int backward) {
-  if (backward) return (size_t)grid_for((int64_t)rows * cols) + 8;
-  return (size_t)((rows + 3) & ~3) + (size_t)(((cols + 255) / 256 + 3) & ~3) + (size_t)((rows + 15) / 16 + 1) * (size_t)cols + 8;
+  return backward ? (size_t)grid_for((int64_t)rows * cols) + 8 : 0;
 }
 
 extern "C" int eadgan_spectral_norm_scale(const float* w_orig, const float* sigma, float* w_sn, long long n,
diff --git a/eadgan_b200/functional.py b/eadgan_b200/functional.py
--- a/eadgan_b200/functional.py
+++ b/eadgan_b200/functional.py
@@ -308,26 +308,43 @@
     return _Upsample2xFn.apply(x)
 
 
-class _SpectralNormFn(torch.autograd.Function):
-
-    @staticmethod
-    def forward(ctx, w_orig, u, v, do_power_iter, eps):
+def spectral_norm_forwards(layers, count, do_power_iter, eps):
+    dev = layers[0][0].device
+    table = (L.SnLayer * len(layers))()
+    keep, outs = [], []
+    for i, (w_orig, u, v) in enumerate(layers):
         _f32(w_orig, "spectral_norm")
-        w = w_orig.contiguous()
+        w = w_orig.detach().contiguous()
         rows = w.shape[0]
         cols = w.numel() // rows
-        sigma = torch.empty(1, device=w.device, dtype=torch.float32)
+        c4 = (count + 3) // 4 * 4
+        buf = torch.empty(c4 + count * (rows + cols), device=dev, dtype=torch.float32)
+        sg = buf[:count]
+        us = buf[c4:c4 + count * rows].view(count, rows)
+        vs = buf[c4 + count * rows:].view(count, cols)
+        table[i] = L.SnLayer(w.data_ptr(), rows, cols, u.data_ptr(), v.data_ptr(), us.data_ptr(), vs.data_ptr(),
+                             sg.data_ptr())
+        keep.append(w)
+        outs.append((us, vs, sg))
+    ws = tc._workspace(L.lib().eadgan_spectral_norm_fwd_workspace(table, len(layers)), dev)
+    call("eadgan_spectral_norm_fwd_multi", table, len(layers), int(count), 1 if do_power_iter else 0, float(eps),
+         ptr(ws), C.c_size_t(ws.numel()), stream())
+    return outs
+
+
+class _SpectralNormFn(torch.autograd.Function):
+
+    @staticmethod
+    def forward(ctx, w_orig, u, v, sigma):
+        w = w_orig.contiguous()
         w_sn = torch.empty_like(w)
-        scratch = torch.empty(L.lib().eadgan_spectral_norm_scratch_floats(rows, cols, 0), device=w.device,
-                              dtype=torch.float32)
-        call("eadgan_spectral_norm_fwd", ptr(w), rows, cols, ptr(u), ptr(v), 1 if do_power_iter else 0,
-             float(eps), ptr(sigma), None if sn_skip_scale else ptr(w_sn), ptr(scratch), stream())
-        ctx.mark_non_differentiable(sigma)
-        ctx.save_for_backward(w, u.clone(), v.clone(), sigma)
-        return w_sn, sigma
-
-    @staticmethod
-    def backward(ctx, dw_sn, _dsigma):
+        if not sn_skip_scale:
+            spectral_norm_materialize(w, sigma, w_sn)
+        ctx.save_for_backward(w, u, v, sigma)
+        return w_sn
+
+    @staticmethod
+    def backward(ctx, dw_sn):
         w, u, v, sigma = ctx.saved_tensors
         dw_sn = dw_sn.contiguous()
         rows = w.shape[0]
@@ -337,7 +354,7 @@
                               dtype=torch.float32)
         call("eadgan_spectral_norm_bwd", ptr(dw_sn), ptr(w), ptr(u), ptr(v), ptr(sigma), rows, cols, ptr(dw),
              ptr(scratch), stream())
-        return dw, None, None, None, None
+        return dw, None, None, None
 
 
 sn_skip_scale = False
@@ -347,8 +364,13 @@
     call("eadgan_spectral_norm_scale", ptr(w_orig.detach().contiguous()), ptr(sigma), ptr(w_sn), w_sn.numel(), stream())
 
 
+def spectral_norm_apply(w_orig, u, v, sigma):
+    return _SpectralNormFn.apply(w_orig, u, v, sigma)
+
+
 def spectral_norm_weight(w_orig, u, v, do_power_iter, eps):
-    return _SpectralNormFn.apply(w_orig, u, v, bool(do_power_iter), float(eps))
+    (us, vs, sg), = spectral_norm_forwards([(w_orig, u, v)], 1, do_power_iter, eps)
+    return spectral_norm_apply(w_orig, us[0], vs[0], sg), sg
 
 
 def _same_shape(a, b, who):
diff --git a/eadgan_b200/tc.py b/eadgan_b200/tc.py
--- a/eadgan_b200/tc.py
+++ b/eadgan_b200/tc.py
@@ -92,15 +92,24 @@
     return _cached_pack(param, "wide", direction, c_alloc)
 
 
+def dense_pack_cached(param, m_pad, rows_major):
+    return _cached_pack(param, "dense", (m_pad, bool(rows_major)), None)
+
+
 def _cached_pack(param, kind, direction, c_alloc):
-    key = (id(param), direction if kind == "wide" else "thin_" + direction, c_alloc)
+    key = (id(param), kind, direction, c_alloc)
     token = (param._version, param.data_ptr(), L.weights_epoch, getattr(param, "_eadgan_stepped", 0))
     _note_use(param, kind, direction, c_alloc)
     hit = _pack_cache.get(key)
     if hit is not None and hit[0]() is param and hit[1] == token:
         return _adopt(hit)
     w = param.detach()
-    out = thin_pack_w(w, direction) if kind == "thin" else pack_w(w, None, direction, c_alloc)
+    if kind == "thin":
+        out = thin_pack_w(w, direction)
+    elif kind == "dense":
+        out = dense_pack(w, *direction)
+    else:
+        out = pack_w(w, None, direction, c_alloc)
     if hit is None or hit[0]() is not param:
         weakref.finalize(param, _pack_cache.pop, key, None)
     _pack_cache[key] = (weakref.ref(param), token, out) + _built_on()
diff --git a/include/eadgan.h b/include/eadgan.h
--- a/include/eadgan.h
+++ b/include/eadgan.h
@@ -146,10 +146,19 @@
 int eadgan_upsample2x_fwd(const float* x, float* y, int nc, int h, int w, void* stream);
 int eadgan_upsample2x_bwd(const float* dy, float* dx, int nc, int h, int w, void* stream);
 
+typedef struct {
+  const float* w;
+  int rows, cols;
+  float* u;
+  float* v;
+  float* u_out;
+  float* v_out;
+  float* sigma_out;
+} EadganSnLayer;
+size_t eadgan_spectral_norm_fwd_workspace(const EadganSnLayer* layers, int n);
+int eadgan_spectral_norm_fwd_multi(const EadganSnLayer* layers, int n, int count, int do_power_iter, float eps,
+                                   void* ws, size_t ws_bytes, void* stream);
 size_t eadgan_spectral_norm_scratch_floats(int rows, int cols, int backward);
-int eadgan_spectral_norm_fwd(const float* w_orig, int rows, int cols, float* u, float* v,
-                             int do_power_iter, float eps, float* sigma, float* w_sn,
-                             float* scratch, void* stream);
 int eadgan_spectral_norm_scale(const float* w_orig, const float* sigma, float* w_sn, long long n, void* stream);
 int eadgan_spectral_norm_bwd(const float* dw_sn, const float* w_orig, const float* u,
                              const float* v, const float* sigma, int rows, int cols,
```

After: 49610 (median of 6 runs). No clear change (-0.1%).
